# jhhung/kISS

Measured on AMD Instinct MI355X. Metric: bases/sec suffix_sort (chm13v2.0-size synthetic, k=256), higher is better.
Workload: dtype u8; 1 GPU; suffix_sort genome-like synthetic n=3117292070 k=256 (stand-in for chm13v2.0.fa, BASELINE.json configs[1]); PARALLEL_SORTING; text resident in HBM, SA left in HBM; n=3117292070, k=256, seed=2, parallelism=single GPU, lms=905939973, lms_rounds=9, tied_after_round0_item_rounds=184319413, big_segment_item_rounds=72866550, workspace_bytes=80357006484, induce_passes=47

## Files before the change

include/kiss_hip.h:

```cpp
#ifndef KISS_HIP_H
#define KISS_HIP_H

#include <stddef.h>
#include <stdint.h>

#ifdef __cplusplus
extern "C" {
#endif

#define KISS_HIP_VERSION 103

typedef enum kiss_hip_status {
    KISS_HIP_OK = 0,
    KISS_HIP_E_INVALID = -1,
    KISS_HIP_E_NO_DEVICE = -2,
    KISS_HIP_E_HIP = -3,
    KISS_HIP_E_NOMEM = -4,
    KISS_HIP_E_UNSUPPORTED = -5,
    KISS_HIP_E_INTERNAL = -6,
    KISS_HIP_E_IO = -7,
    KISS_HIP_E_DEEP = -8
} kiss_hip_status;

#define KISS_HIP_ALGO_PARALLEL_SORTING 0
// ... 75 lines not shown
int kiss_hip_release_cached_contexts(void);

int kiss_hip_ctx_suffix_sort_dna_u32(kiss_hip_ctx *ctx, const uint8_t *S, uint64_t n, uint32_t k, int algo,
                                     uint32_t *SA);

int kiss_hip_ctx_suffix_sort_dna_u32_dev(kiss_hip_ctx *ctx, const uint8_t *d_S, uint64_t n, uint32_t k, int algo,
                                         uint32_t *d_SA, void *stream);

typedef struct kiss_hip_multi kiss_hip_multi;
typedef struct kiss_hip_multi_stats {
    uint64_t n, m;
    uint32_t ndev;
    uint32_t refine_depth;
    uint64_t piece[8];
    float ms_total, ms_pack, ms_classify, ms_partition, ms_exchange, ms_sort, ms_gather, ms_induce;
} kiss_hip_multi_stats;
int kiss_hip_multi_create(kiss_hip_multi **out, const int *devices, int ndev, uint64_t max_n);
int kiss_hip_multi_destroy(kiss_hip_multi *mc);
int kiss_hip_multi_suffix_sort_dna_u32(kiss_hip_multi *mc, const uint8_t *S, uint64_t n, uint32_t k, int algo, uint32_t *SA);
int kiss_hip_multi_suffix_sort_dna_u32_dev(kiss_hip_multi *mc, const uint8_t *d_S, uint64_t n, uint32_t k, int algo,
                                           uint32_t *d_SA);
int kiss_hip_multi_get_stats(const kiss_hip_multi *mc, kiss_hip_multi_stats *out);
kiss_hip_ctx *kiss_hip_multi_ctx(kiss_hip_multi *mc, int rank);
int kiss_hip_suffix_sort_dna_u32_multi(const uint8_t *S, uint64_t n, uint32_t k, int algo, uint32_t *SA, const int *devices,
                                       int ndev);

typedef struct kiss_hip_verify_report {
    uint64_t n;
    uint32_t k;
    uint32_t exact;
    uint32_t ok;
    uint32_t sa0_ok;
    uint64_t out_of_range;
    uint64_t duplicates;
    uint64_t order_violations;
    uint64_t first_violation;
    uint64_t tied_pairs;
    uint64_t digest;
    float ms;
    uint32_t reserved_;
} kiss_hip_verify_report;
int kiss_hip_ctx_verify_sa_dev(kiss_hip_ctx *ctx, const uint8_t *d_S, uint64_t n, uint32_t k, const uint32_t *d_SA,
                               kiss_hip_verify_report *out, void *stream);
uint64_t kiss_hip_sa_digest_host(const uint32_t *SA, uint64_t count);
uint64_t kiss_hip_fnv1a64_host(const void *data, uint64_t bytes, uint64_t seed);

int kiss_hip_ctx_get_stage_outputs(kiss_hip_ctx *ctx, uint32_t *lms_ascending, uint32_t *lms_sorted,
                                   uint64_t *counts);

int kiss_hip_stage_classify(kiss_hip_ctx *ctx, const uint8_t *d_S, uint64_t n, uint32_t k, uint64_t lo, uint64_t hi,
                            uint64_t counts13[13], void *stream);
int kiss_hip_stage_local_lms(kiss_hip_ctx *ctx, uint64_t *d_keys_out ,
                             uint32_t *d_pos_out, uint64_t *m_local, uint64_t *m_far_local);
enum {
    KISS_HIP_VIEW_LOCAL_KEYS = 0,
    KISS_HIP_VIEW_LOCAL_POS = 1,
    KISS_HIP_VIEW_PART_KEYS = 2,
    KISS_HIP_VIEW_PART_POS = 3,
    KISS_HIP_VIEW_SORTED = 4,
    KISS_HIP_VIEW_SORTED_CTX = 5
};
int kiss_hip_stage_view(kiss_hip_ctx *ctx, int which, void **d_ptr, uint64_t *capacity);
int kiss_hip_stage_reserve(kiss_hip_ctx *ctx, uint64_t lms_capacity);
int kiss_hip_stage_key_hist(kiss_hip_ctx *ctx, const uint64_t *d_keys, uint64_t count, int bits, uint64_t *d_hist,
                            void *stream);
int kiss_hip_stage_partition(kiss_hip_ctx *ctx, const uint64_t *d_keys, const uint32_t *d_pos, uint64_t count, int bits,
                             const uint32_t *splitters, int groups, uint64_t *d_keys_out, uint32_t *d_pos_out,
                             void *stream);
int kiss_hip_stage_sort(kiss_hip_ctx *ctx, const uint64_t *d_keys, const uint32_t *d_pos, uint64_t count, uint64_t n,
                        uint32_t k, uint32_t *d_sorted_out, uint32_t *d_ctx_out, void *stream);
int kiss_hip_stage_induce(kiss_hip_ctx *ctx, uint64_t n, uint32_t k, const uint32_t *d_far_sorted,
                          const uint32_t *d_far_ctx, uint64_t m_far, const uint32_t *d_near_pos, uint64_t near_count,
                          const uint64_t counts12[12], uint32_t *d_SA, void *stream);
int kiss_hip_stage_induce_exact(kiss_hip_ctx *ctx, uint64_t n, uint32_t h0, const uint32_t *d_far_sorted,
                                const uint32_t *d_far_ctx, uint64_t m_far, const uint32_t *d_near_pos, uint64_t near_count,
                                const uint64_t counts12[12], uint32_t *d_SA, void *stream, int *exact_out);
int kiss_hip_stage_refine_exact(kiss_hip_ctx *ctx, uint64_t n, uint32_t h0, uint32_t *d_SA, void *stream);

int kiss_hip_debug_radix_sort(kiss_hip_ctx *ctx, uint64_t *keys, uint32_t *pos, uint64_t count, int key_lo_bit);
int kiss_hip_debug_radix_sort_seg(kiss_hip_ctx *ctx, uint64_t *keys, uint32_t *seg, uint32_t *pos, uint64_t count,
                                  int key_lo_bit, int seg_bits, unsigned flags);
int kiss_hip_debug_scan_u32(kiss_hip_ctx *ctx, uint32_t *data, uint64_t count);
int kiss_hip_debug_fail_alloc_over(kiss_hip_ctx *ctx, uint64_t bytes);
int kiss_hip_debug_splitters(const uint64_t *hist, uint64_t bins, int groups, uint32_t *splitters_out,
                             uint64_t *group_counts_out);

typedef struct kiss_hip_fmi_view {
    uint64_t n_sa;
    uint32_t cnt[4];
    uint32_t pri;
    uint32_t sa_intv;
    const uint8_t *bwt;
    const uint32_t *occ1;
    const uint8_t *occ2;
    const uint32_t *sa;
    const uint64_t *b;
    const uint32_t *b_occ;
} kiss_hip_fmi_view;

int kiss_hip_fmi_query_batch_dev(kiss_hip_ctx *ctx, const kiss_hip_fmi_view *fmi, const uint8_t *patterns, uint32_t L,
                                 uint64_t Q, uint32_t *beg, uint32_t *end, uint64_t *hit_count_total,
                                 uint64_t *checksum, uint32_t *offsets, uint64_t *offsets_index,
                                 uint64_t offsets_capacity, void *stream);

int kiss_hip_fmi_build_dev(kiss_hip_ctx *ctx, const uint8_t *d_S, uint64_t n, const uint32_t *d_SA, uint32_t sa_intv,
                           uint8_t *d_bwt, uint32_t *d_occ1, uint8_t *d_occ2, uint32_t *d_sa_sampled, uint64_t *d_b,
                           uint32_t *d_b_occ, uint32_t cnt_out[4], uint32_t *pri_out, void *stream);

typedef struct kiss_hip_fmi_sizes {
    uint64_t n_sa, bwt_bytes, occ1_entries, occ2_bytes, sa_entries, b_words, b_occ_entries;
} kiss_hip_fmi_sizes;
int kiss_hip_fmi_sizes_for(uint64_t n, kiss_hip_fmi_sizes *out);
int kiss_hip_fmi_build_host(const uint8_t *S, uint64_t n, const uint32_t *SA_or_null, uint8_t *bwt, uint32_t *occ1,
                            uint8_t *occ2, uint32_t *sa, uint64_t *b, uint32_t *b_occ, uint32_t cnt_out[4],
                            uint32_t *pri_out, int device);
int kiss_hip_fmi_query_batch_host(const kiss_hip_fmi_view *fmi, const uint8_t *patterns, uint32_t L, uint64_t Q,
                                  uint32_t *beg, uint32_t *end, uint64_t *hit_count_total, uint64_t *checksum,
                                  uint32_t *offsets, uint64_t *offsets_index, uint64_t offsets_capacity, int device);

#define KISS_HIP_FMI_MAX_SA_INTV 32u
#define KISS_HIP_FMI_MAX_LOOKUP_LEN 14u
typedef struct kiss_hip_fmi_view_ex {
    kiss_hip_fmi_view base;
    uint32_t lookup_len;
    const uint32_t *lookup;
} kiss_hip_fmi_view_ex;
typedef struct kiss_hip_fmi_sizes_ex {
    kiss_hip_fmi_sizes base;
    uint64_t lookup_entries;
} kiss_hip_fmi_sizes_ex;
int kiss_hip_fmi_sizes_ex_for(uint64_t n, uint32_t sa_intv, uint32_t lookup_len, kiss_hip_fmi_sizes_ex *out);
int kiss_hip_fmi_build_ex_dev(kiss_hip_ctx *ctx, const uint8_t *d_S, uint64_t n, const uint32_t *d_SA, uint32_t sa_intv,
                              uint32_t lookup_len, uint8_t *d_bwt, uint32_t *d_occ1, uint8_t *d_occ2, uint32_t *d_sa,
                              uint64_t *d_b, uint32_t *d_b_occ, uint32_t *d_lookup, uint32_t cnt_out[4], uint32_t *pri_out,
                              void *stream);
int kiss_hip_fmi_query_ex_dev(kiss_hip_ctx *ctx, const kiss_hip_fmi_view_ex *fmi, const uint8_t *patterns, uint32_t L,
                              uint64_t Q, uint32_t stop_cnt, uint32_t *beg, uint32_t *end, uint32_t *offs,
                              uint64_t *hit_count_total, uint64_t *checksum, uint32_t *offsets, uint64_t *offsets_index,
                              uint64_t offsets_capacity, void *stream);
int kiss_hip_fmi_build_ex_host(const uint8_t *S, uint64_t n, const uint32_t *SA_or_null, uint32_t sa_intv,
                               uint32_t lookup_len, uint8_t *bwt, uint32_t *occ1, uint8_t *occ2, uint32_t *sa, uint64_t *b,
                               uint32_t *b_occ, uint32_t *lookup, uint32_t cnt_out[4], uint32_t *pri_out, int device);
int kiss_hip_fmi_query_ex_host(const kiss_hip_fmi_view_ex *fmi, const uint8_t *patterns, uint32_t L, uint64_t Q,
                               uint32_t stop_cnt, uint32_t *beg, uint32_t *end, uint32_t *offs, uint64_t *hit_count_total,
                               uint64_t *checksum, uint32_t *offsets, uint64_t *offsets_index, uint64_t offsets_capacity,
                               int device);

#define KISS_HIP_FMI_MAX_MISMATCHES 3u
typedef struct kiss_hip_fmi_mm_report {
    uint64_t Q;
    uint32_t L, max_mismatches;
    uint64_t hits[4];
    uint64_t ranges;
    uint64_t lf_pairs;
    uint64_t walk_failures;
    uint64_t checksum;
    float ms_total, ms_search, ms_locate, ms_sort;
} kiss_hip_fmi_mm_report;
int kiss_hip_fmi_query_mm_dev(kiss_hip_ctx *ctx, const kiss_hip_fmi_view *fmi, const uint8_t *patterns, uint32_t L, uint64_t Q,
                              uint32_t max_mismatches, uint32_t *counts, uint32_t *positions, uint8_t *mismatches,
                              uint64_t *index, uint64_t capacity, kiss_hip_fmi_mm_report *report, void *stream);
int kiss_hip_fmi_query_mm_host(const kiss_hip_fmi_view *fmi, const uint8_t *patterns, uint32_t L, uint64_t Q,
                               uint32_t max_mismatches, uint32_t *counts, uint32_t *positions, uint8_t *mismatches,
                               uint64_t *index, uint64_t capacity, kiss_hip_fmi_mm_report *report, int device);

int kiss_hip_suffix_sort_u8(const uint8_t *S, uint64_t n, uint32_t *SA, int device);
// ... 207 lines not shown
```

kiss_amd/_lib.py:

```python
import ctypes
import os

_HERE = os.path.dirname(os.path.abspath(__file__))
LIB_PATH = os.path.join(_HERE, "libkiss_hip.so")
HOOKS_LIB_PATH = os.path.join(_HERE, "libkiss_hip_hooks.so")

KISS_HIP_OK = 0
KISS_HIP_E_INVALID, KISS_HIP_E_NO_DEVICE, KISS_HIP_E_HIP, KISS_HIP_E_NOMEM = -1, -2, -3, -4
KISS_HIP_E_UNSUPPORTED, KISS_HIP_E_INTERNAL, KISS_HIP_E_IO, KISS_HIP_E_DEEP = -5, -6, -7, -8
ALGO_PARALLEL_SORTING = 0
ALGO_PREFIX_DOUBLING = 1
MAX_N = 4294963200
VIEW_LOCAL_KEYS, VIEW_LOCAL_POS, VIEW_PART_KEYS, VIEW_PART_POS, VIEW_SORTED, VIEW_SORTED_CTX = range(6)

KERNEL_CLASSES = [
    "pack", "classify", "radix_hist", "radix_scatter", "scan", "keygather", "flag_compact",
    "place", "induce_count", "induce_scatter", "induce_small", "fm_query", "fm_build", "segrank",
    "group_heads", "isa",
]


class Report(ctypes.Structure):

    def as_dict(self):
# ... 265 lines not shown

class InsertReport(Report):
    _fields_ = [(k, ctypes.c_uint64) for k in ("P", "unmapped", "bad_input", "low_mapq", "discordant", "too_long", "samples", "used")] + [
        (k, ctypes.c_uint32) for k in ("flags", "q25", "q50", "q75", "mean", "sd", "ins_min", "ins_max", "ins_mean")] + [
        ("ms_total", ctypes.c_float), ("ms_hist", ctypes.c_float), ("ms_stats", ctypes.c_float),
    ]


class Fmi8View(ctypes.Structure):
    _fields_ = [
        ("n_sa", ctypes.c_uint64), ("pri", ctypes.c_uint32), ("sa_intv", ctypes.c_uint32), ("sigma", ctypes.c_uint32),
        ("reserved_", ctypes.c_uint32), ("C", ctypes.c_void_p), ("map", ctypes.c_void_p), ("bwt", ctypes.c_void_p),
        ("occ1", ctypes.c_void_p), ("occ2", ctypes.c_void_p), ("sa", ctypes.c_void_p), ("b", ctypes.c_void_p),
        ("b_occ", ctypes.c_void_p),
    ]


class Fmi8Sizes(Report):
    _fields_ = [(k, ctypes.c_uint64) for k in ("n_sa", "bwt_bytes", "occ1_entries", "occ2_entries", "sa_entries", "b_words",
                                               "b_occ_entries")]


class Fmi8Report(Report):
    _fields_ = [
        ("Q", ctypes.c_uint64), ("hits", ctypes.c_uint64), ("lf_pairs", ctypes.c_uint64), ("walk_failures", ctypes.c_uint64),
        ("checksum", ctypes.c_uint64), ("ms_total", ctypes.c_float), ("ms_search", ctypes.c_float),
        ("ms_locate", ctypes.c_float), ("ms_sort", ctypes.c_float),
    ]


class KissHipError(RuntimeError):
    def __init__(self, status, where, detail=""):
        self.status = status
        msg = "%s failed: %s (%d)" % (where, strerror(status), status)
        if detail:
            msg += " [" + detail + "]"
        super().__init__(msg)


_libs = {}


def load(hooks=None):
    if hooks is None:
        hooks = os.environ.get("KISS_AMD_LIB", "") == "hooks"
    hooks = bool(hooks)
    if hooks in _libs:
        return _libs[hooks]
    path = HOOKS_LIB_PATH if hooks else LIB_PATH
    if not hooks and os.environ.get("KISS_AMD_LIB_PATH"):
        path = os.environ["KISS_AMD_LIB_PATH"]
    if not os.path.exists(path):
        raise ImportError(
            "%s not built at %s -- run `python -c 'import __graft_entry__ as g; g.build()'` "
            "or `make -C kiss_amd/csrc`; there is no CPU fallback" % (os.path.basename(path), path))
    lib = ctypes.CDLL(path)
    if hasattr(lib, "kiss_hip_has_hooks"):
        lib.kiss_hip_has_hooks.restype = ctypes.c_int
        if bool(lib.kiss_hip_has_hooks()) != hooks and not os.environ.get("KISS_AMD_LIB_PATH"):
            raise ImportError("%s is not the %s build" % (path, "hooks" if hooks else "default"))
    elif hooks:
        raise ImportError("%s is not a hooks build" % path)
    vp, u8p = ctypes.c_void_p, ctypes.c_void_p
    lib.kiss_hip_version.restype = ctypes.c_int
    lib.kiss_hip_strerror.restype = ctypes.c_char_p
    lib.kiss_hip_strerror.argtypes = [ctypes.c_int]
    lib.kiss_hip_device_count.argtypes = [ctypes.POINTER(ctypes.c_int)]
    lib.kiss_hip_ctx_create.argtypes = [ctypes.POINTER(vp), ctypes.c_int, ctypes.c_uint64]
    lib.kiss_hip_ctx_create_sized.argtypes = [ctypes.POINTER(vp), ctypes.c_int, ctypes.c_uint64, ctypes.c_uint64]
    lib.kiss_hip_ctx_release_io_buffers.argtypes = [vp]
    ip = ctypes.POINTER(ctypes.c_int)
    lib.kiss_hip_multi_create.argtypes = [ctypes.POINTER(vp), ip, ctypes.c_int, ctypes.c_uint64]
    lib.kiss_hip_multi_destroy.argtypes = [vp]
    lib.kiss_hip_multi_suffix_sort_dna_u32.argtypes = [vp, vp, ctypes.c_uint64, ctypes.c_uint32, ctypes.c_int, vp]
    lib.kiss_hip_multi_suffix_sort_dna_u32_dev.argtypes = [vp, vp, ctypes.c_uint64, ctypes.c_uint32, ctypes.c_int, vp]
    lib.kiss_hip_multi_get_stats.argtypes = [vp, ctypes.POINTER(MultiStats)]
    lib.kiss_hip_multi_ctx.argtypes = [vp, ctypes.c_int]
    lib.kiss_hip_multi_ctx.restype = vp
    lib.kiss_hip_suffix_sort_dna_u32_multi.argtypes = [vp, ctypes.c_uint64, ctypes.c_uint32, ctypes.c_int, vp, ip, ctypes.c_int]
    lib.kiss_hip_stage_view.argtypes = [vp, ctypes.c_int, ctypes.POINTER(vp), ctypes.POINTER(ctypes.c_uint64)]
    lib.kiss_hip_stage_reserve.argtypes = [vp, ctypes.c_uint64]
    lib.kiss_hip_debug_fail_alloc_over.argtypes = [vp, ctypes.c_uint64]
    lib.kiss_hip_debug_fail_alloc_over.restype = ctypes.c_int
    lib.kiss_hip_debug_splitters.argtypes = [vp, ctypes.c_uint64, ctypes.c_int, vp, vp]
    lib.kiss_hip_debug_splitters.restype = ctypes.c_int
    lib.kiss_hip_ctx_destroy.argtypes = [vp]
    lib.kiss_hip_ctx_set_profiling.argtypes = [vp, ctypes.c_int]
    lib.kiss_hip_ctx_set_profiling_mask.argtypes = [vp, ctypes.c_uint64]
    lib.kiss_hip_last_hip_error.argtypes = [vp, ctypes.POINTER(ctypes.c_char_p)]
    lib.kiss_hip_get_stats.argtypes = [vp, ctypes.POINTER(Stats)]
    lib.kiss_hip_ctx_workspace_bytes.argtypes = [vp, ctypes.POINTER(ctypes.c_uint64)]
    lib.kiss_hip_suffix_sort_dna_u32.argtypes = [u8p, ctypes.c_uint64, ctypes.c_uint32, ctypes.c_int, vp, ctypes.c_int]
    lib.kiss_hip_ctx_suffix_sort_dna_u32.argtypes = [vp, u8p, ctypes.c_uint64, ctypes.c_uint32, ctypes.c_int, vp]
    lib.kiss_hip_ctx_suffix_sort_dna_u32_dev.argtypes = [vp, vp, ctypes.c_uint64, ctypes.c_uint32, ctypes.c_int, vp, vp]
    lib.kiss_hip_ctx_get_stage_outputs.argtypes = [vp, vp, vp, vp]
    lib.kiss_hip_ctx_verify_sa_dev.argtypes = [vp, vp, ctypes.c_uint64, ctypes.c_uint32, vp, ctypes.POINTER(VerifyReport), vp]
    lib.kiss_hip_ctx_verify_sa_dev.restype = ctypes.c_int
    lib.kiss_hip_sa_digest_host.argtypes = [vp, ctypes.c_uint64]
    lib.kiss_hip_sa_digest_host.restype = ctypes.c_uint64
    lib.kiss_hip_fnv1a64_host.argtypes = [vp, ctypes.c_uint64, ctypes.c_uint64]
    lib.kiss_hip_fnv1a64_host.restype = ctypes.c_uint64
    lib.kiss_hip_debug_radix_sort.argtypes = [vp, vp, vp, ctypes.c_uint64, ctypes.c_int]
    lib.kiss_hip_debug_radix_sort_seg.argtypes = [vp, vp, vp, vp, ctypes.c_uint64, ctypes.c_int, ctypes.c_int, ctypes.c_uint]
    lib.kiss_hip_debug_radix_sort_seg.restype = ctypes.c_int
    lib.kiss_hip_debug_scan_u32.argtypes = [vp, vp, ctypes.c_uint64]
    u64 = ctypes.c_uint64
    lib.kiss_hip_stage_classify.argtypes = [vp, vp, u64, ctypes.c_uint32, u64, u64, ctypes.POINTER(u64 * 13), vp]
    lib.kiss_hip_stage_local_lms.argtypes = [vp, vp, vp, ctypes.POINTER(u64), ctypes.POINTER(u64)]
    lib.kiss_hip_stage_key_hist.argtypes = [vp, vp, u64, ctypes.c_int, vp, vp]
    lib.kiss_hip_stage_partition.argtypes = [vp, vp, vp, u64, ctypes.c_int, vp, ctypes.c_int, vp, vp, vp]
    lib.kiss_hip_stage_sort.argtypes = [vp, vp, vp, u64, u64, ctypes.c_uint32, vp, vp, vp]
    lib.kiss_hip_stage_induce.argtypes = [vp, u64, ctypes.c_uint32, vp, vp, u64, vp, u64, ctypes.POINTER(u64 * 12), vp, vp]
    lib.kiss_hip_stage_induce_exact.argtypes = [vp, u64, ctypes.c_uint32, vp, vp, u64, vp, u64, ctypes.POINTER(u64 * 12), vp, vp,
                                                ctypes.POINTER(ctypes.c_int)]
    lib.kiss_hip_stage_refine_exact.argtypes = [vp, u64, ctypes.c_uint32, vp, vp]
    lib.kiss_hip_stage_refine_exact.restype = ctypes.c_int
    lib.kiss_hip_fmi_query_batch_dev.argtypes = [
        vp, ctypes.POINTER(FmiView), vp, ctypes.c_uint32, ctypes.c_uint64, vp, vp,
        ctypes.POINTER(ctypes.c_uint64), ctypes.POINTER(ctypes.c_uint64), vp, vp, ctypes.c_uint64, vp]
    lib.kiss_hip_fmi_build_dev.argtypes = [
        vp, vp, ctypes.c_uint64, vp, ctypes.c_uint32, vp, vp, vp, vp, vp, vp,
        ctypes.POINTER(ctypes.c_uint32 * 4), ctypes.POINTER(ctypes.c_uint32), vp]
    u32 = ctypes.c_uint32
    lib.kiss_hip_fmi_sizes_ex_for.argtypes = [u64, u32, u32, ctypes.POINTER(FmiSizesEx)]
    lib.kiss_hip_fmi_build_ex_dev.argtypes = [
        vp, vp, u64, vp, u32, u32, vp, vp, vp, vp, vp, vp, vp, ctypes.POINTER(u32 * 4), ctypes.POINTER(u32), vp]
    lib.kiss_hip_fmi_query_ex_dev.argtypes = [
        vp, ctypes.POINTER(FmiViewEx), vp, u32, u64, u32, vp, vp, vp, ctypes.POINTER(u64), ctypes.POINTER(u64), vp, vp,
        u64, vp]
    lib.kiss_hip_fmi_build_ex_host.argtypes = [vp, u64, vp, u32, u32] + [vp] * 9 + [ctypes.c_int]
    lib.kiss_hip_fmi_query_ex_host.argtypes = [ctypes.POINTER(FmiViewEx), vp, u32, u64, u32, vp, vp, vp,
                                               ctypes.POINTER(u64), ctypes.POINTER(u64), vp, vp, u64, ctypes.c_int]
    lib.kiss_hip_fmi_query_mm_dev.argtypes = [vp, ctypes.POINTER(FmiView), vp, u32, u64, u32, vp, vp, vp, vp, u64,
                                              ctypes.POINTER(FmiMmReport), vp]
    lib.kiss_hip_fmi_query_mm_host.argtypes = [ctypes.POINTER(FmiView), vp, u32, u64, u32, vp, vp, vp, vp, u64,
                                               ctypes.POINTER(FmiMmReport), ctypes.c_int]
    lib.kiss_hip_fmi_query_mm_dev.restype = lib.kiss_hip_fmi_query_mm_host.restype = ctypes.c_int
    lib.kiss_hip_fmi_seeds_dev.argtypes = [vp, ctypes.POINTER(FmiViewEx), vp, vp, u64, u32, u32, u32, ctypes.c_int, vp, vp, vp, u64,
                                           vp, vp, u64, ctypes.POINTER(FmiSeedReport), vp]
    lib.kiss_hip_fmi_seeds_host.argtypes = [ctypes.POINTER(FmiViewEx), vp, vp, u64, u32, u32, u32, ctypes.c_int, vp, vp, vp, u64,
                                            vp, vp, u64, ctypes.POINTER(FmiSeedReport), ctypes.c_int]
    lib.kiss_hip_fmi_seeds_dev.restype = lib.kiss_hip_fmi_seeds_host.restype = ctypes.c_int
    lib.kiss_hip_fmi_chain_dev.argtypes = [vp, vp, vp, u64, vp, vp, ctypes.POINTER(ChainParams), vp, vp, u64, vp, vp, u64,
                                           ctypes.POINTER(ChainReport), vp]
    lib.kiss_hip_fmi_chain_host.argtypes = [vp, vp, u64, vp, vp, ctypes.POINTER(ChainParams), vp, vp, u64, vp, vp, u64,
                                            ctypes.POINTER(ChainReport), ctypes.c_int]
    lib.kiss_hip_fmi_chain_dev.restype = lib.kiss_hip_fmi_chain_host.restype = ctypes.c_int
    lib.kiss_hip_fmi_align_dev.argtypes = [vp, vp, u64, vp, vp, u64, ctypes.c_int, vp, vp, ctypes.POINTER(AlignParams), vp, u64, vp,
                                           vp, u64, ctypes.POINTER(AlignReport), vp]
    lib.kiss_hip_fmi_align_host.argtypes = [vp, u64, vp, vp, u64, ctypes.c_int, vp, vp, ctypes.POINTER(AlignParams), vp, u64, vp, vp,
                                            u64, ctypes.POINTER(AlignReport), ctypes.c_int]
    lib.kiss_hip_fmi_align_dev.restype = lib.kiss_hip_fmi_align_host.restype = ctypes.c_int
    lib.kiss_hip_fmi_select_dev.argtypes = [vp, vp, vp, vp, u64, ctypes.c_int, vp, u64, ctypes.POINTER(SelectParams), vp, vp, u64,
                                            ctypes.POINTER(SelectReport), vp]
    lib.kiss_hip_fmi_select_host.argtypes = [vp, vp, vp, u64, ctypes.c_int, vp, u64, ctypes.POINTER(SelectParams), vp, vp, u64,
                                             ctypes.POINTER(SelectReport), ctypes.c_int]
    lib.kiss_hip_fmi_select_dev.restype = lib.kiss_hip_fmi_select_host.restype = ctypes.c_int
    lib.kiss_hip_fmi_pair_dev.argtypes = [vp, vp, vp, u64, vp, u64, ctypes.POINTER(PairParams), vp, ctypes.POINTER(PairReport), vp]
    lib.kiss_hip_fmi_pair_host.argtypes = [vp, vp, u64, vp, u64, ctypes.POINTER(PairParams), vp, ctypes.POINTER(PairReport),
                                           ctypes.c_int]
    lib.kiss_hip_fmi_pair_dev.restype = lib.kiss_hip_fmi_pair_host.restype = ctypes.c_int
    lib.kiss_hip_fmi_rescue_dev.argtypes = [vp, vp, vp, vp, u64, vp, u64, vp, u64, vp, u64, ctypes.POINTER(RescueParams), vp, vp, vp, u64,
                                            ctypes.POINTER(RescueReport), vp]
    lib.kiss_hip_fmi_rescue_host.argtypes = [vp, vp, vp, u64, vp, u64, vp, u64, vp, u64, ctypes.POINTER(RescueParams), vp, vp, vp, u64,
                                             ctypes.POINTER(RescueReport), ctypes.c_int]
    lib.kiss_hip_fmi_rescue_dev.restype = lib.kiss_hip_fmi_rescue_host.restype = ctypes.c_int
# ... 52 lines not shown
            getattr(lib, name).restype = ctypes.c_int
    lib.kiss_hip_fmi_insert_dev.argtypes = [vp, vp, vp, u64, vp, u64, ctypes.POINTER(InsertParams), vp, ctypes.POINTER(InsertReport), vp]
    lib.kiss_hip_fmi_insert_host.argtypes = [vp, vp, u64, vp, u64, ctypes.POINTER(InsertParams), vp, ctypes.POINTER(InsertReport),
                                             ctypes.c_int]
    for name in INSERT_EXPORTED_SYMBOLS:
        getattr(lib, name).restype = ctypes.c_int
    lib.kiss_hip_fmi8_sizes_for.argtypes = [u64, u32, u32, ctypes.POINTER(Fmi8Sizes)]
    lib.kiss_hip_fmi8_build_dev.argtypes = [vp, vp, u64, vp, u32, u32] + [vp] * 8 + [ctypes.POINTER(u32), ctypes.POINTER(u32), vp]
    lib.kiss_hip_fmi8_build_host.argtypes = [vp, u64, vp, u32, u32] + [vp] * 8 + [ctypes.POINTER(u32), ctypes.POINTER(u32),
                                                                                  ctypes.c_int]
    lib.kiss_hip_fmi8_query_dev.argtypes = [vp, ctypes.POINTER(Fmi8View), vp, vp, u64, vp, vp, ctypes.POINTER(u64),
                                            ctypes.POINTER(u64), vp, vp, u64, ctypes.POINTER(Fmi8Report), vp]
    lib.kiss_hip_fmi8_query_host.argtypes = [ctypes.POINTER(Fmi8View), vp, vp, u64, vp, vp, ctypes.POINTER(u64),
                                             ctypes.POINTER(u64), vp, vp, u64, ctypes.POINTER(Fmi8Report), ctypes.c_int]
    for name in ("kiss_hip_fmi8_sizes_for", "kiss_hip_fmi8_build_dev", "kiss_hip_fmi8_build_host", "kiss_hip_fmi8_query_dev",
                 "kiss_hip_fmi8_query_host"):
        getattr(lib, name).restype = ctypes.c_int
    lib.kiss_hip_file_size.argtypes = [ctypes.c_char_p, ctypes.POINTER(u64)]
    lib.kiss_hip_ctx_parse_text_dev.argtypes = [vp, vp, u64, vp, ctypes.POINTER(u64), vp]
    lib.kiss_hip_ctx_load_text_file.argtypes = [vp, ctypes.c_char_p, ctypes.POINTER(vp), ctypes.POINTER(u64)]
    lib.kiss_hip_copy_to_host.argtypes = [vp, vp, u64]
    lib.kiss_hip_suffix_sort_u8.argtypes = [vp, u64, vp, ctypes.c_int]
    lib.kiss_hip_suffix_sort_u8.restype = ctypes.c_int
    lib.kiss_hip_ctx_suffix_sort_u8_dev.argtypes = [vp, vp, u64, vp, vp]
    lib.kiss_hip_ctx_suffix_sort_u8_dev.restype = ctypes.c_int
    lib.kiss_hip_free_dev.argtypes = [vp]
    lib.kiss_hip_alloc_dev.argtypes = [ctypes.POINTER(vp), u64]
    lib.kiss_hip_alloc_dev.restype = ctypes.c_int
    for name in ("kiss_hip_ctx_lcp_dna_u32_dev", "kiss_hip_ctx_lcp_u8_dev"):
        getattr(lib, name).argtypes = [vp, vp, u64, vp, vp, ctypes.POINTER(LcpReport), vp]
        getattr(lib, name).restype = ctypes.c_int
    for name in ("kiss_hip_lcp_dna_u32", "kiss_hip_lcp_u8"):
        getattr(lib, name).argtypes = [vp, u64, vp, vp, vp, ctypes.c_int]
        getattr(lib, name).restype = ctypes.c_int
    for name in ("kiss_hip_file_size", "kiss_hip_ctx_parse_text_dev", "kiss_hip_ctx_load_text_file",
                 "kiss_hip_copy_to_host", "kiss_hip_free_dev"):
        getattr(lib, name).restype = ctypes.c_int
    for name in ("kiss_hip_device_count", "kiss_hip_ctx_create", "kiss_hip_ctx_destroy", "kiss_hip_ctx_set_profiling", "kiss_hip_ctx_set_profiling_mask",
                 "kiss_hip_last_hip_error", "kiss_hip_get_stats", "kiss_hip_ctx_workspace_bytes",
                 "kiss_hip_suffix_sort_dna_u32", "kiss_hip_ctx_suffix_sort_dna_u32",
                 "kiss_hip_ctx_suffix_sort_dna_u32_dev", "kiss_hip_ctx_get_stage_outputs",
                 "kiss_hip_fmi_query_batch_dev", "kiss_hip_fmi_build_dev", "kiss_hip_debug_radix_sort",
                 "kiss_hip_debug_scan_u32", "kiss_hip_stage_classify", "kiss_hip_stage_local_lms",
                 "kiss_hip_stage_key_hist", "kiss_hip_stage_partition", "kiss_hip_stage_sort", "kiss_hip_stage_induce",
                 "kiss_hip_ctx_create_sized", "kiss_hip_ctx_release_io_buffers", "kiss_hip_multi_create",
                 "kiss_hip_multi_destroy", "kiss_hip_multi_suffix_sort_dna_u32", "kiss_hip_multi_suffix_sort_dna_u32_dev",
                 "kiss_hip_multi_get_stats", "kiss_hip_suffix_sort_dna_u32_multi", "kiss_hip_stage_view",
                 "kiss_hip_stage_reserve", "kiss_hip_fmi_sizes_ex_for", "kiss_hip_fmi_build_ex_dev",
                 "kiss_hip_fmi_query_ex_dev", "kiss_hip_fmi_build_ex_host", "kiss_hip_fmi_query_ex_host"):
        getattr(lib, name).restype = ctypes.c_int
    _libs[hooks] = lib
    return lib


def strerror(status):
    return load().kiss_hip_strerror(int(status)).decode()


EXPORTED_SYMBOLS = [
    "kiss_hip_version", "kiss_hip_strerror", "kiss_hip_device_count", "kiss_hip_ctx_create", "kiss_hip_ctx_destroy",
    "kiss_hip_ctx_set_profiling", "kiss_hip_ctx_set_profiling_mask", "kiss_hip_last_hip_error", "kiss_hip_get_stats", "kiss_hip_ctx_workspace_bytes",
    "kiss_hip_suffix_sort_dna_u32", "kiss_hip_ctx_suffix_sort_dna_u32", "kiss_hip_ctx_suffix_sort_dna_u32_dev",
    "kiss_hip_ctx_get_stage_outputs", "kiss_hip_ctx_verify_sa_dev", "kiss_hip_sa_digest_host", "kiss_hip_fnv1a64_host",
    "kiss_hip_fmi_query_batch_dev", "kiss_hip_fmi_build_dev",
    "kiss_hip_debug_radix_sort", "kiss_hip_debug_radix_sort_seg", "kiss_hip_debug_scan_u32",
    "kiss_hip_stage_classify", "kiss_hip_stage_local_lms", "kiss_hip_stage_key_hist", "kiss_hip_stage_partition",
    "kiss_hip_stage_sort", "kiss_hip_stage_induce", "kiss_hip_stage_induce_exact", "kiss_hip_stage_refine_exact",
    "kiss_hip_fmi_sizes_for", "kiss_hip_fmi_build_host", "kiss_hip_fmi_query_batch_host",
    "kiss_hip_file_size", "kiss_hip_ctx_parse_text_dev", "kiss_hip_ctx_load_text_file", "kiss_hip_copy_to_host",
    "kiss_hip_free_dev", "kiss_hip_alloc_dev", "kiss_hip_suffix_sort_u8", "kiss_hip_ctx_suffix_sort_u8_dev",
    "kiss_hip_ctx_create_sized", "kiss_hip_ctx_release_io_buffers", "kiss_hip_stage_view", "kiss_hip_stage_reserve",
    "kiss_hip_multi_create", "kiss_hip_multi_destroy", "kiss_hip_multi_suffix_sort_dna_u32",
    "kiss_hip_multi_suffix_sort_dna_u32_dev", "kiss_hip_multi_get_stats", "kiss_hip_multi_ctx",
    "kiss_hip_suffix_sort_dna_u32_multi", "kiss_hip_debug_splitters", "kiss_hip_debug_fail_alloc_over",
    "kiss_hip_has_hooks", "kiss_hip_release_cached_contexts", "kiss_hip_get_stats_sized",
    "kiss_hip_fmi_sizes_ex_for", "kiss_hip_fmi_build_ex_dev", "kiss_hip_fmi_query_ex_dev", "kiss_hip_fmi_build_ex_host",
    "kiss_hip_fmi_query_ex_host", "kiss_hip_ctx_lcp_dna_u32_dev", "kiss_hip_ctx_lcp_u8_dev", "kiss_hip_lcp_dna_u32",
    "kiss_hip_lcp_u8", "kiss_hip_fmi_query_mm_dev", "kiss_hip_fmi_query_mm_host",
    "kiss_hip_fmi8_sizes_for", "kiss_hip_fmi8_build_dev", "kiss_hip_fmi8_build_host", "kiss_hip_fmi8_query_dev",
    "kiss_hip_fmi8_query_host", "kiss_hip_fmi_seeds_dev", "kiss_hip_fmi_seeds_host",
    "kiss_hip_fmi_chain_dev", "kiss_hip_fmi_chain_host", "kiss_hip_fmi_align_dev", "kiss_hip_fmi_align_host",
    "kiss_hip_fmi_select_dev", "kiss_hip_fmi_select_host", "kiss_hip_fmi_pair_dev", "kiss_hip_fmi_pair_host",
    "kiss_hip_fmi_rescue_dev", "kiss_hip_fmi_rescue_host", "kiss_hip_fmi_aln_merge_dev", "kiss_hip_fmi_aln_merge_host",
]

READS_EXPORTED_SYMBOLS = [
    "kiss_hip_reads_parse_dev", "kiss_hip_reads_parse_host", "kiss_hip_reads_interleave_dev", "kiss_hip_reads_interleave_host",
]
READS_PART_EXPORTED_SYMBOLS = ["kiss_hip_reads_parse_part_dev", "kiss_hip_reads_parse_part_host"]
MD_EXPORTED_SYMBOLS = ["kiss_hip_fmi_md_dev", "kiss_hip_fmi_md_host"]
PILEUP_EXPORTED_SYMBOLS = ["kiss_hip_fmi_pileup_dev", "kiss_hip_fmi_pileup_host"]
PILEUP_PLANES = 8
SAM_EXPORTED_SYMBOLS = ["kiss_hip_fmi_sam_dev", "kiss_hip_fmi_sam_host"]
BAM_EXPORTED_SYMBOLS = ["kiss_hip_fmi_bam_dev", "kiss_hip_fmi_bam_host", "kiss_hip_bgzf_dev", "kiss_hip_bgzf_host"]
BGZF_BLOCK_DEFAULT, BGZF_BLOCK_MAX, BGZF_OVERHEAD, BGZF_EOF_BYTES = 65280, 65505, 31, 28
DEFLATE_EXPORTED_SYMBOLS = ["kiss_hip_bgzf_deflate_dev", "kiss_hip_bgzf_deflate_host"]
BAM_SORT_EXPORTED_SYMBOLS = ["kiss_hip_bam_sort_dev", "kiss_hip_bam_sort_host"]
BAM_RECORD_MIN = 36
BAI_EXPORTED_SYMBOLS = ["kiss_hip_bai_dev", "kiss_hip_bai_host"]
BAI_PSEUDO_BIN, BAI_MAX_END = 37450, 1 << 29
INSERT_EXPORTED_SYMBOLS = ["kiss_hip_fmi_insert_dev", "kiss_hip_fmi_insert_host"]
INSERT_MAX = 65535
INSERT_OK = 1
READS_AUTO, READS_LINES, READS_FASTQ = 0, 1, 2
READS_NONE = 0xFFFFFFFFFFFFFFFF
```

kiss_amd/csrc/api.hip:

```cpp
#include "kiss_internal.hpp"
#include <cstdlib>
#include <chrono>
#include <mutex>
#include <cstring>
#include <new>

KTimer::KTimer(kiss_hip_ctx *c, int cls, uint64_t items) : ctx(c), idx(-1)
{
    if (!((ctx->profile_mask >> cls) & 1ull)) return;
    if (ctx->ev_used == ctx->ev_pool.size()) {
        kiss_hip_ctx::Ev e;
        if (hipEventCreate(&e.a) != hipSuccess || hipEventCreate(&e.b) != hipSuccess) return;
        e.cls = 0;
        ctx->ev_pool.push_back(e);
    }
    idx = (int)ctx->ev_used++;
    ctx->ev_pool[idx].cls = cls;
    ctx->stats.launches_kernel[cls]++;
    ctx->stats.items_kernel[cls] += items;
    (void)hipEventRecord(ctx->ev_pool[idx].a, ctx->stream);
}
KTimer::~KTimer()
{
    if (idx >= 0) (void)hipEventRecord(ctx->ev_pool[idx].b, ctx->stream);
}
void ktimer_collect(kiss_hip_ctx *ctx)
{
    for (size_t i = 0; i < ctx->ev_used; i++) {
        float ms = 0.f;
        if (hipEventElapsedTime(&ms, ctx->ev_pool[i].a, ctx->ev_pool[i].b) == hipSuccess)
            ctx->stats.ms_kernel[ctx->ev_pool[i].cls] += ms;
    }
    ctx->ev_used = 0;
}

static void kiss_opts_supported_from_env(KissOpts &o)
{
    o.debug = getenv("KISS_HIP_DEBUG") != nullptr;
    if (const char *e = getenv("KISS_HIP_XFER_THREADS")) o.xfer_threads = atoi(e);
    if (const char *e = getenv("KISS_HIP_PREFAULT_THREADS")) o.prefault_threads = atoi(e);
}
#ifdef KISS_HIP_HOOKS
static bool env_on(const char *name) { return getenv(name) != nullptr; }
static unsigned long long env_u64(const char *name, unsigned long long dflt)
{
    const char *e = getenv(name);
    return e ? strtoull(e, nullptr, 0) : dflt;
}
void kiss_opts_refresh(kiss_hip_ctx *ctx)
{
    KissOpts o;
    kiss_opts_supported_from_env(o);
    if (const char *e = getenv("KISS_HIP_SYNC_READBACK")) o.sync_readback = atoi(e) != 0;
    o.no_serialize = env_on("KISS_HIP_NO_SERIALIZE");
    o.no_lms_exact = env_on("KISS_HIP_NO_LMS_EXACT");
    o.heads_by_compare = env_on("KISS_HIP_LMS_HEADS_BY_COMPARE");
    o.no_early_out = env_on("KISS_HIP_NO_EARLY_OUT");
    o.no_pivot_rounds = env_on("KISS_HIP_NO_PIVOT_ROUNDS");
    o.pivot_from_round2 = env_on("KISS_HIP_PIVOT_FROM_ROUND2");
    o.pair_keys = env_on("KISS_HIP_PAIR_KEYS");
    o.no_fc0_onepass = env_on("KISS_HIP_NO_FC0_ONEPASS");
    o.no_pair_records = env_on("KISS_HIP_NO_PAIR_RECORDS");
    o.no_small_fused = env_on("KISS_HIP_NO_SMALL_FUSED");
    o.no_class_bytes = env_on("KISS_HIP_NO_CLASS_BYTES");
    o.no_pivot_ctx = env_on("KISS_HIP_NO_PIVOT_CTX");
    o.no_taint = env_on("KISS_HIP_NO_TAINT");
    o.isa_direct = env_on("KISS_HIP_ISA_DIRECT");
    o.no_onesweep = env_on("KISS_HIP_NO_ONESWEEP");
    o.rx_one_tile = env_on("KISS_HIP_RX_ONE_TILE");
    o.merge_lms = env_on("KISS_HIP_MERGE_LMS");
    o.no_small_alphabet = env_on("KISS_HIP_NO_SMALL_ALPHABET");
    o.induce_one_pass = env_on("KISS_HIP_INDUCE_ONE_PASS");
    o.verify = env_on("KISS_HIP_VERIFY");
    o.no_prefault = env_on("KISS_HIP_NO_PREFAULT");
    o.doubling_h0 = (uint32_t)env_u64("KISS_HIP_DOUBLING_H0", 0);
    o.tcap0 = env_u64("KISS_HIP_TCAP0", 0);
    o.pivot_slots = (int)env_u64("KISS_HIP_PIVOT_SLOTS", 3);
    o.small_seg = (uint32_t)env_u64("KISS_HIP_SMALL_SEG", 0);
    o.near_merge_min = (uint32_t)env_u64("KISS_HIP_NEAR_MERGE_MIN", 4096);
    o.induce_small_max = (uint32_t)env_u64("KISS_HIP_INDUCE_SMALL_MAX", 0);
    o.collapse_cap = (uint32_t)env_u64("KISS_HIP_COLLAPSE_CAP", 0);
    o.collapse_n = env_u64("KISS_HIP_COLLAPSE_N", 0);
    o.fm_heavy = (uint32_t)env_u64("KISS_HIP_FM_HEAVY", 0);
    o.fm_light = (uint32_t)env_u64("KISS_HIP_FM_LIGHT", 0);
    o.fm_mm_wave = env_on("KISS_HIP_FM_MM_WAVE");
    o.fm_mm_budget = env_u64("KISS_HIP_FM_MM_BUDGET", 0);
    o.fm8_group = env_on("KISS_HIP_FM8_GROUP");
    o.isa_direct_max = env_u64("KISS_HIP_ISA_DIRECT_MAX", 0);
    o.lx_sync_points = (unsigned)env_u64("KISS_HIP_LX_SYNC_POINTS", 0);
    o.tie_trace = (unsigned)env_u64("KISS_HIP_TIE_TRACE", 0);
    o.poison = (uint32_t)env_u64("KISS_HIP_POISON", 0);
    if (const char *e = getenv("KISS_HIP_DUMP_PIVOT")) snprintf(o.dump_pivot, sizeof o.dump_pivot, "%s", e);
    ctx->opts = o;
}
static std::mutex &kiss_launch_mutex()
{
    static std::mutex m;
    return m;
}
static bool kiss_lock_launches()
{
    static const bool on = getenv("KISS_HIP_LOCK_LAUNCHES") != nullptr;
    return on;
}
bool kiss_sync_launches()
{
    static const bool on = getenv("KISS_HIP_SYNC_LAUNCHES") != nullptr;
    return on;
}
KissLaunchGuard::KissLaunchGuard() : held(kiss_lock_launches())
{
    if (held) kiss_launch_mutex().lock();
}
KissLaunchGuard::~KissLaunchGuard()
{
    if (held) kiss_launch_mutex().unlock();
}
#endif

std::mutex &kiss_device_mutex(int device)
{
    static std::mutex m[64];
    return m[(unsigned)device & 63u];
}

__global__ void k_publish(const uint32_t *__restrict__ src, uint32_t nwords, uint32_t *host_dst, uint32_t seq)
{
    const uint32_t t = threadIdx.x;
    if (t < nwords) __hip_atomic_store(&host_dst[t], src[t], __ATOMIC_RELAXED, __HIP_MEMORY_SCOPE_SYSTEM);
    __threadfence_system();
    if (t == 0) __hip_atomic_store(&host_dst[16], seq, __ATOMIC_RELEASE, __HIP_MEMORY_SCOPE_SYSTEM);
}

int kiss_readback(kiss_hip_ctx *ctx, const void *d_src, uint32_t nwords)
{
    if (nwords > 16) return KINTERNAL();
    ctx->pub_mode = ctx->opts.sync_readback || !ctx->h_pub || !ctx->d_pub ? 0 : 1;
    if (ctx->pub_mode == 0) {
        KCHECK(hipMemcpyAsync(ctx->h_pinned, d_src, nwords * sizeof(uint32_t), hipMemcpyDeviceToHost, ctx->stream));
        KCHECK(hipStreamSynchronize(ctx->stream));
        return KISS_HIP_OK;
    }
    const uint32_t seq = ++ctx->pub_seq ? ctx->pub_seq : ++ctx->pub_seq;
    hipLaunchKernelGGL(k_publish, dim3(1), dim3(64), 0, ctx->stream, (const uint32_t *)d_src, nwords, ctx->d_pub, seq);
    KCHECK(hipGetLastError());
    volatile uint32_t *flag = ctx->h_pub + 16;
    const auto t0 = std::chrono::steady_clock::now();
    for (uint64_t spins = 0;; spins++) {
        if (__atomic_load_n(flag, __ATOMIC_ACQUIRE) == seq) break;
#if defined(__x86_64__) || defined(__i386__)
        __builtin_ia32_pause();
#endif
        if ((spins & 0xFFFF) == 0xFFFF) {
            const double s = std::chrono::duration<double>(std::chrono::steady_clock::now() - t0).count();
            if (s > 5.0) {
                KCHECK(hipStreamSynchronize(ctx->stream));
                if (__atomic_load_n(flag, __ATOMIC_ACQUIRE) != seq) return KINTERNAL();
                break;
            }
        }
    }
    for (uint32_t i = 0; i < nwords; i++) ctx->h_pinned[i] = ctx->h_pub[i];
    return KISS_HIP_OK;
}

bool kiss_host_is_pinned(const void *p);
void *kiss_prefault_start(kiss_hip_ctx *ctx, void *p, uint64_t bytes);
void kiss_prefault_join(void *handle);

void kiss_drain_deferred(kiss_hip_ctx *ctx)
{
    for (void *p : ctx->deferred_free) (void)hipFree(p);
    ctx->deferred_free.clear();
    ctx->deferred_bytes = 0;
}

namespace {

template <typename T>
int dmalloc(kiss_hip_ctx *ctx, T **p, uint64_t count)
{
    void *q = nullptr;
    uint64_t bytes = (count ? count : 1) * sizeof(T);
    hipError_t e = ctx->fail_alloc_over && bytes > ctx->fail_alloc_over ? hipErrorOutOfMemory : hipMalloc(&q, bytes);
#ifdef KISS_HIP_HOOKS
    if (e == hipSuccess && ctx->opts.poison) e = hipMemsetD32(q, (int)ctx->opts.poison, bytes / 4);
#endif
    if (e != hipSuccess) {
        (void)hipGetLastError();
        ctx->last_hip_error = (int)e;
        return KISS_HIP_E_NOMEM;
    }
    ctx->ws_bytes += bytes;
    *p = reinterpret_cast<T *>(q);
    return KISS_HIP_OK;
}

void release(kiss_hip_ctx *ctx, void *p, bool defer)
{
    if (defer) ctx->deferred_free.push_back(p);
    else (void)hipFree(p);
}

void free_tied(kiss_hip_ctx *ctx, bool defer = false)
{
    void **ptrs[] = {(void **)&ctx->segA, (void **)&ctx->segB, (void **)&ctx->slotA, (void **)&ctx->slotB,
                     (void **)&ctx->segstartA, (void **)&ctx->segstartB, (void **)&ctx->bkeyA, (void **)&ctx->bkeyB,
                     (void **)&ctx->bposA, (void **)&ctx->bposB, (void **)&ctx->bsegA, (void **)&ctx->bsegB,
                     (void **)&ctx->bslot, (void **)&ctx->flags};
    for (void **p : ptrs)
        if (*p) {
            release(ctx, *p, defer);
            *p = nullptr;
        }
    if (defer) ctx->deferred_bytes += ctx->tied_bytes;
    ctx->ws_bytes -= ctx->tied_bytes;
    ctx->tied_bytes = 0;
    ctx->t_cap = 0;
    ctx->flags_cap = 0;
}

void free_lms_side(kiss_hip_ctx *ctx, bool defer = false)
{
    free_tied(ctx, defer);
    void **ptrs[] = {(void **)&ctx->lms_pos, (void **)&ctx->keyA, (void **)&ctx->keyB, (void **)&ctx->posA,
                     (void **)&ctx->posB, (void **)&ctx->lms_sorted_far, (void **)&ctx->lms_ctx_far,
                     (void **)&ctx->lmsP, (void **)&ctx->lmsC, (void **)&ctx->tile_hist, (void **)&ctx->scan_tmp,
                     (void **)&ctx->rx_desc, (void **)&ctx->rx_ghist, (void **)&ctx->fc_desc};
    for (void **p : ptrs)
        if (*p) {
            release(ctx, *p, defer);
            *p = nullptr;
        }
    if (defer) ctx->deferred_bytes += ctx->lms_bytes;
    ctx->ws_bytes -= ctx->lms_bytes;
    ctx->lms_bytes = 0;
}

void free_all(kiss_hip_ctx *ctx)
{
    kiss_drain_deferred(ctx);
    free_lms_side(ctx);
    void *ptrs[] = {ctx->pk, ctx->tile_gp, ctx->tile_cnt, ctx->cl_part, ctx->d_counts, ctx->CTX, ctx->CLS, ctx->ind_counts, ctx->ind_desc,
                    ctx->d_small, ctx->near_idx, ctx->near_fin, ctx->near_pos, ctx->near_tmp, ctx->near_tmp2, ctx->pairs1, ctx->pairs2, ctx->rx_ctl, ctx->refine_heads, ctx->ga_codes};
    for (void *p : ptrs)
        if (p) (void)hipFree(p);
    for (void *p : ctx->fm_pool)
        if (p) (void)hipFree(p);
    for (hipEvent_t e : ctx->fm_ev)
        if (e) (void)hipEventDestroy(e);
#ifdef KISS_HIP_HOOKS
    if (ctx->tie_dbg) (void)hipFree(ctx->tie_dbg);
#endif
    if (ctx->io_S) (void)hipFree(ctx->io_S);
    if (ctx->io_SA) (void)hipFree(ctx->io_SA);
    kiss_xfer_free(ctx);
    if (ctx->h_pinned) (void)hipHostFree(ctx->h_pinned);
    if (ctx->h_pub) (void)hipHostFree(ctx->h_pub);
    for (auto &e : ctx->ev_pool) {
        (void)hipEventDestroy(e.a);
        (void)hipEventDestroy(e.b);
    }
    if (ctx->own_stream) (void)hipStreamDestroy(ctx->own_stream);
}

int sort_dev_unlocked(kiss_hip_ctx *ctx, const uint8_t *d_S, uint64_t n, uint32_t k, int algo, uint32_t *d_SA, void *stream);
int sort_dev(kiss_hip_ctx *ctx, const uint8_t *d_S, uint64_t n, uint32_t k, int algo, uint32_t *d_SA, void *stream)
{
    if (!ctx) return KISS_HIP_E_INVALID;
    kiss_opts_refresh(ctx);
#ifdef KISS_NO_DEVICE_LOCK
    return sort_dev_unlocked(ctx, d_S, n, k, algo, d_SA, stream);
#endif
    if (ctx->opts.no_serialize) return sort_dev_unlocked(ctx, d_S, n, k, algo, d_SA, stream);
    std::lock_guard<std::mutex> lock(kiss_device_mutex(ctx->device));
    return sort_dev_unlocked(ctx, d_S, n, k, algo, d_SA, stream);
}
int sort_dev_unlocked(kiss_hip_ctx *ctx, const uint8_t *d_S, uint64_t n, uint32_t k, int algo, uint32_t *d_SA, void *stream)
{
    if (!ctx || !d_SA || (n && !d_S)) return KISS_HIP_E_INVALID;
    if (n > KISS_HIP_MAX_N || n > ctx->max_n) return KISS_HIP_E_INVALID;
    if (algo != KISS_HIP_ALGO_PARALLEL_SORTING && algo != KISS_HIP_ALGO_PREFIX_DOUBLING) return KISS_HIP_E_INVALID;
    KCHECK(hipSetDevice(ctx->device));
    KissCallStream call_stream(ctx, stream);
    KTRY(kiss_workspace_ready(ctx));
    std::memset(&ctx->stats, 0, sizeof ctx->stats);
    ctx->stats.n = n;
    ctx->stats.k = k;
    ctx->n = n;
    ctx->m = ctx->m_far = 0;
    if (n == 0) {
        KTRY(kiss_zero_u32(ctx, d_SA, 1));
        KCHECK(hipStreamSynchronize(ctx->stream));
        return KISS_HIP_OK;
    }
    uint64_t depth;
    if ((uint64_t)k >= n) depth = 0;
    else depth = (uint64_t)KISS_STRIDE * ((uint64_t)k / KISS_STRIDE + 1);
    if (algo == KISS_HIP_ALGO_PREFIX_DOUBLING && depth != 0) {
        algo = KISS_HIP_ALGO_PARALLEL_SORTING;
    }
    ctx->stats.depth = (uint32_t)(depth > 0xFFFFFFFFull ? 0xFFFFFFFFull : depth);
    uint32_t h0 = 0;
    if (algo == KISS_HIP_ALGO_PREFIX_DOUBLING) {
        h0 = KISS_EXACT_H0;
        if (ctx->opts.doubling_h0 >= 32 && ctx->opts.doubling_h0 <= (1u << 20)) h0 = ctx->opts.doubling_h0;
        if (n < 4ull * h0 + 1024) h0 = 0;
        else {
            k = h0;
            depth = (uint64_t)KISS_STRIDE * ((uint64_t)k / KISS_STRIDE + 1);
        }
    }
    ctx->stats.refine_depth = h0;

    hipEvent_t ev[8];
    for (auto &e : ev) KCHECK(hipEventCreate(&e));
    const bool lms_exact = !ctx->opts.no_lms_exact;
    int rc = KISS_HIP_OK;
    for (int attempt = 0; attempt < 2; attempt++) {
        (void)hipEventRecord(ev[0], ctx->stream);
        if ((rc = kiss_pack_text(ctx, d_S, n))) break;
        (void)hipEventRecord(ev[1], ctx->stream);
        if ((rc = kiss_classify(ctx, n, depth, 0, n))) break;
        (void)hipEventRecord(ev[2], ctx->stream);
        ctx->hfar = nullptr;
        ctx->h_depth = h0;
// ... 262 lines not shown
    ctx->stats.ms_d2h = std::chrono::duration<float, std::milli>(t3 - t2).count();
    return KISS_HIP_OK;
}

int kiss_io_release(kiss_hip_ctx *ctx)
{
    if (ctx->io_S) (void)hipFree(ctx->io_S);
    if (ctx->io_SA) (void)hipFree(ctx->io_SA);
    ctx->io_S = nullptr;
    ctx->io_SA = nullptr;
    ctx->ws_bytes -= ctx->io_cap ? 5 * ctx->io_cap + 4 : 0;
    ctx->io_cap = 0;
    return KISS_HIP_OK;
}

extern "C" {

int kiss_hip_version(void) { return KISS_HIP_VERSION; }

const char *kiss_hip_strerror(int status)
{
    switch (status) {
    case KISS_HIP_OK: return "ok";
    case KISS_HIP_E_INVALID: return "invalid argument";
    case KISS_HIP_E_NO_DEVICE: return "no usable HIP device";
    case KISS_HIP_E_HIP: return "HIP runtime error";
    case KISS_HIP_E_NOMEM: return "out of memory";
    case KISS_HIP_E_UNSUPPORTED: return "request outside the implemented range";
    case KISS_HIP_E_INTERNAL: return "internal invariant violated";
    case KISS_HIP_E_IO: return "file could not be opened or read";
    case KISS_HIP_E_DEEP: return "ties deeper than the bounded-round exact path handles: sort with a bounded k, then stage_refine_exact";
    default: return "unknown status";
    }
}

int kiss_hip_device_count(int *count)
{
    if (!count) return KISS_HIP_E_INVALID;
    int c = 0;
    if (hipGetDeviceCount(&c) != hipSuccess) {
        *count = 0;
        return KISS_HIP_E_NO_DEVICE;
    }
    *count = c;
    return KISS_HIP_OK;
}

int kiss_hip_ctx_create(kiss_hip_ctx **out, int device, uint64_t max_n)
{
    return kiss_hip_ctx_create_sized(out, device, max_n, 0);
}

int kiss_hip_ctx_create_sized(kiss_hip_ctx **out, int device, uint64_t max_n, uint64_t lms_capacity)
{
    if (!out || max_n > KISS_HIP_MAX_N) return KISS_HIP_E_INVALID;
    *out = nullptr;
    int ndev = 0;
    if (hipGetDeviceCount(&ndev) != hipSuccess || ndev <= 0 || device < 0 || device >= ndev) return KISS_HIP_E_NO_DEVICE;
    kiss_hip_ctx *ctx = new (std::nothrow) kiss_hip_ctx();
    if (!ctx) return KISS_HIP_E_NOMEM;
    ctx->device = device;
    ctx->max_n = max_n;
    ctx->m_cap0 = lms_capacity ? lms_capacity + 4096 : 0;
    kiss_opts_supported_from_env(ctx->opts);
    kiss_opts_refresh(ctx);
    int rc = KISS_HIP_OK;
    do {
        if (hipSetDevice(device) != hipSuccess || hipStreamCreate(&ctx->own_stream) != hipSuccess) {
            rc = KISS_HIP_E_HIP;
            break;
        }
        ctx->stream = ctx->own_stream;
        const uint64_t words = max_n / 32 + 8;
        ctx->pk_words = words;
        ctx->n_tiles_cap = words / 256 + 2;
        ctx->ind_tiles_cap = 4 * ((max_n + 1) / 1024 + 2) + 2;
#define ALLOC(p, cnt) if ((rc = dmalloc(ctx, &ctx->p, (cnt)))) break
        ALLOC(pk, words);
        ALLOC(tile_gp, ctx->n_tiles_cap);
        ALLOC(tile_cnt, ctx->n_tiles_cap);
        ALLOC(cl_part, (ctx->n_tiles_cap < 8192 ? ctx->n_tiles_cap : 8192) * (uint64_t)(KISS_R0_PASSES * 256));
        ALLOC(d_counts, 16);
        ALLOC(ind_counts, ctx->ind_tiles_cap);
        ctx->ind_desc_stride = (max_n + 1) / 1024 + 2;
        ALLOC(ind_desc, 4 * ctx->ind_desc_stride);
        if (hipMemset(ctx->ind_desc, 0, 4 * ctx->ind_desc_stride * sizeof(uint64_t)) != hipSuccess) {
            rc = KISS_HIP_E_HIP;
            break;
        }
        ALLOC(rx_ctl, 4);
        if (hipMemset(ctx->rx_ctl, 0, 4 * sizeof(uint32_t)) != hipSuccess) {
            rc = KISS_HIP_E_HIP;
            break;
        }

        ALLOC(d_small, 64);
#undef ALLOC
        if ((rc = kiss_lms_reserve(ctx, default_m_cap(ctx)))) break;
        void *hp = nullptr;
        if (hipHostMalloc(&hp, 64 * sizeof(uint32_t), hipHostMallocDefault) != hipSuccess) {
            rc = KISS_HIP_E_NOMEM;
            break;
        }
        ctx->h_pinned = reinterpret_cast<uint32_t *>(hp);
        void *pub = nullptr, *dpub = nullptr;
        if (hipHostMalloc(&pub, 32 * sizeof(uint32_t), hipHostMallocCoherent | hipHostMallocMapped) == hipSuccess) {
            std::memset(pub, 0, 32 * sizeof(uint32_t));
            if (hipHostGetDevicePointer(&dpub, pub, 0) == hipSuccess) {
                ctx->h_pub = reinterpret_cast<uint32_t *>(pub);
                ctx->d_pub = reinterpret_cast<uint32_t *>(dpub);
            } else {
                (void)hipHostFree(pub);
            }
        }
        (void)hipGetLastError();
    } while (0);
    if (rc != KISS_HIP_OK) {
        free_all(ctx);
        delete ctx;
        return rc;
    }
    *out = ctx;
    return KISS_HIP_OK;
}

int kiss_hip_ctx_destroy(kiss_hip_ctx *ctx)
{
    if (!ctx) return KISS_HIP_E_INVALID;
    (void)hipSetDevice(ctx->device);
    free_all(ctx);
    delete ctx;
    return KISS_HIP_OK;
}

int kiss_hip_ctx_set_profiling(kiss_hip_ctx *ctx, int enabled)
{
    if (!ctx) return KISS_HIP_E_INVALID;
    ctx->profile_mask = enabled ? ~0ull : 0ull;
    return KISS_HIP_OK;
}

int kiss_hip_ctx_set_profiling_mask(kiss_hip_ctx *ctx, uint64_t class_mask)
{
    if (!ctx) return KISS_HIP_E_INVALID;
    ctx->profile_mask = class_mask;
    return KISS_HIP_OK;
}

int kiss_hip_last_hip_error(const kiss_hip_ctx *ctx, const char **msg)
{
    if (!ctx) return 0;
    if (msg) *msg = hipGetErrorString((hipError_t)ctx->last_hip_error);
    return ctx->last_hip_error;
}

int kiss_hip_get_stats(const kiss_hip_ctx *ctx, kiss_hip_stats *out)
{
    if (!ctx || !out) return KISS_HIP_E_INVALID;
    *out = ctx->stats;
    return KISS_HIP_OK;
}

int kiss_hip_get_stats_sized(const kiss_hip_ctx *ctx, void *out, uint64_t bytes)
{
    if (!ctx || !out) return KISS_HIP_E_INVALID;
    const uint64_t have = sizeof ctx->stats;
// ... 222 lines not shown
```

kiss_amd/csrc/induce.hip:

```cpp
#include "kiss_internal.hpp"
#include "induce_count.hpp"
#include <cstdio>
#include <cstdlib>

namespace {

constexpr int IN_THREADS = 256;
#ifndef KISS_IN_ITEMS
#define KISS_IN_ITEMS 8
#endif
constexpr int IN_ITEMS = KISS_IN_ITEMS;
constexpr int IN_WAVES = IN_THREADS / 64;
constexpr int IN_TILE = IN_THREADS * IN_ITEMS;
constexpr int SM_THREADS = 1024;
constexpr uint64_t SMALL_MAX = 8192;

__device__ __forceinline__ uint32_t child_ctx(uint32_t parent)
{
    return (KISS_CTX_WORD(parent) >> 2) | (parent & KISS_CTX_TAINT);
}

__device__ __forceinline__ uint32_t cls_byte(uint32_t c)
{
    return (c & 3u) | ((c & 0x7FFFFFFEu) == 0u ? 4u : 0u);
// ... 160 lines not shown
        const int nb = (int)mis - 4 * (int)lane;
        const uint32_t lowmask = nb >= 4 ? 0xFFFFFFFFu : (nb <= 0 ? 0u : ~(0xFFFFFFFFu << (8 * (nb & 3))));
        w[8] = (w[8] & lowmask) | (0x08080808u & ~lowmask);
    }
    KissClsAcc acc = {{0u, 0u, 0u, 0u}};
    uint32_t any = 0;
#pragma unroll
    for (int i = 0; i < 8; i++) {
        kiss_cls_acc_add(acc, w[i]);
        any |= w[i];
    }
    if (mis != 0u) {
        kiss_cls_acc_add(acc, w[8]);
        any |= w[8];
    }
    uint32_t cnt8 = kiss_cls_acc_sum(acc);
    if (__ballot((any & 0x04040404u) != 0u) != 0ull) {
        uint64_t pend = 0;
#pragma unroll
        for (int i = 0; i < 9; i++) {
            const uint32_t p = (w[i] >> 2) & ~(w[i] >> 3) & 0x01010101u;
            pend |= (uint64_t)(((p * 0x00204081u) >> 21) & 0xFu) << (4 * i);
        }
        cnt8 = refresh_pending<4>(pk, srcP, srcC, srcK, pend, first + 16 * (int64_t)lane, 1024, first + 2048 + 4 * (int64_t)lane,
                                  cnt8, false);
    }
    put_counts(counts, tiles, tile, kiss_cls_emit(cnt8, emitmask));
}

__device__ __forceinline__ void count_word_tile(const uint64_t *__restrict__ pk, const uint32_t *srcP, uint32_t *srcC, int64_t beg,
                                                int dir, uint32_t emitmask, uint32_t *__restrict__ counts, uint64_t tiles,
                                                uint64_t tile, int64_t shift)
{
    struct __attribute__((packed, aligned(4))) U4 {
        uint32_t v[4];
    };
    constexpr int STEPS = IN_TILE / 256;
    static_assert(STEPS * 4 == 32, "one bit per item of a lane in the low half of refresh_pending's mask");
    static_assert(IN_TILE / 64 <= 255, "8-bit counters per lane");
    const uint64_t i0 = tile * IN_TILE + 4 * lane_id();
    const int64_t p0 = (dir > 0 ? beg + (int64_t)i0 : beg - (int64_t)(i0 + 3)) - shift;
    const int64_t pstep = dir > 0 ? 256 : -256;
    U4 t[STEPS];
#pragma unroll
    for (int q = 0; q < STEPS; q++) t[q] = *reinterpret_cast<const U4 *>(srcC + (p0 + q * pstep));
    uint32_t cnt8 = 0, least = 0xFFFFFFFFu;
#pragma unroll
    for (int q = 0; q < STEPS; q++) {
#pragma unroll
        for (int e = 0; e < 4; e++) {
            cnt8 += 1u << ((t[q].v[e] << 3) & 31u);
            least = min(least, t[q].v[e] & 0x7FFFFFFEu);
        }
    }
    if (__ballot(least == 0u) != 0ull) {
        uint32_t pend = 0;
#pragma unroll
        for (int q = 0; q < STEPS; q++)
#pragma unroll
            for (int e = 0; e < 4; e++) pend |= ((t[q].v[e] & 0x7FFFFFFEu) == 0u ? 1u : 0u) << (4 * q + e);
        cnt8 = refresh_pending<2>(pk, srcP, srcC, nullptr, (uint64_t)pend, p0, pstep, 0, cnt8, true);
    }
    put_counts(counts, tiles, tile, kiss_cls_emit(cnt8, emitmask));
}

template <bool REMAP>
__device__ __forceinline__ void count_partial_tile(const uint64_t *__restrict__ pk, const uint32_t *srcP, uint32_t *srcC, int64_t beg,
                                                   uint64_t N, int dir, uint32_t emitmask, uint32_t *__restrict__ counts,
                                                   uint64_t tiles, uint64_t tile, const LmsRemap &rm, uint8_t *srcK)
{
    const uint64_t t0 = tile * IN_TILE;
    uint32_t cnt8 = 0;
    for (uint64_t i = t0 + lane_id(); i < N && i < t0 + IN_TILE; i += 64) {
        const uint32_t cls = item_class_only<REMAP>(pk, srcP, srcC, beg + (int64_t)dir * (int64_t)i, emitmask, rm, REMAP ? nullptr : srcK);
        cnt8 += (cls < 4u ? 1u : 0u) << ((cls & 3u) << 3);
    }
    put_counts(counts, tiles, tile, cnt8);
}

template <bool REMAP>
__global__ __launch_bounds__(IN_THREADS) void k_induce_count(const uint64_t *__restrict__ pk, const uint32_t *srcP,
                                                            uint32_t *srcC, int64_t beg, uint64_t N, int dir,
                                                            uint32_t emitmask, uint32_t *__restrict__ counts,
                                                            uint64_t tiles, LmsRemap rm, uint8_t *srcK)
{
    if (blockIdx.x == 0 && threadIdx.x == 4) counts[4 * tiles] = 0;
    const uint32_t wave = (uint32_t)__builtin_amdgcn_readfirstlane((int)(threadIdx.x >> 6));
    const uint64_t tile = (uint64_t)blockIdx.x * IN_WAVES + wave;
    if (tile >= tiles) return;
    const uint64_t t0 = tile * IN_TILE;
    int64_t shift = 0;
    bool block = t0 + IN_TILE <= N;
    if (REMAP && block) {
        const uint32_t b0 = remap_below_wave(rm, (uint64_t)beg + t0);
        block = b0 == remap_below_wave(rm, (uint64_t)beg + t0 + IN_TILE);
        shift = (int64_t)b0;
    }
    if (!block) count_partial_tile<REMAP>(pk, srcP, srcC, beg, N, dir, emitmask, counts, tiles, tile, rm, srcK);
    else if (!REMAP && srcK != nullptr) count_byte_tile(pk, srcP, srcC, srcK, beg, dir, emitmask, counts, tiles, tile);
    else count_word_tile(pk, srcP, srcC, beg, dir, emitmask, counts, tiles, tile, shift);
}

struct DstPos {
    int64_t p[4];
};

template <bool REMAP, int DIR>
__global__ __launch_bounds__(IN_THREADS) void k_induce_scatter(const uint64_t *__restrict__ pk, const uint32_t *srcP,
                                                              uint32_t *srcC, int64_t beg, uint64_t N,
                                                              uint32_t emitmask, const uint32_t *__restrict__ ex,
                                                              uint64_t tiles, DstPos dst, uint32_t *SA, uint32_t *CTX,
                                                              uint32_t *__restrict__ totals, LmsRemap rm,
                                                              uint8_t *CLS,
                                                              uint8_t *srcK)
{
    static_assert(IN_ITEMS == 8 && IN_WAVES == 4, "8-bit counters per thread, 4-bit ranks of a thread's items in one word");
    static_assert(!REMAP || DIR > 0, "the LMS list is read left to right only");
    __shared__ uint32_t wtot[IN_WAVES][2];
    __shared__ __attribute__((aligned(16))) uint32_t stP[IN_TILE];
    __shared__ __attribute__((aligned(16))) uint32_t stC[IN_TILE];
    if (blockIdx.x == 0 && threadIdx.x < 4) totals[threadIdx.x] = ex[(uint64_t)(threadIdx.x + 1) * tiles] - ex[(uint64_t)threadIdx.x * tiles];
    const int wave = threadIdx.x >> 6;
    struct __attribute__((packed, aligned(4))) U4 {
        uint32_t v[4];
    };
    const uint64_t i0 = (uint64_t)blockIdx.x * IN_TILE + (uint64_t)threadIdx.x * IN_ITEMS;
    uint32_t vv[IN_ITEMS], cc[IN_ITEMS];
    uint32_t okm = 0;
    uint32_t loc = 0;
    uint32_t cnt8 = 0;
    auto take = [&](int e, uint32_t pc, uint32_t ok) {
        const uint32_t sh = pc << 3;
        loc |= ((cnt8 >> sh) & 15u) << (4 * e);
        cnt8 += ok << sh;
        okm |= ok << e;
    };
    int64_t shift = 0;
    bool block = i0 + IN_ITEMS <= N;
    if (REMAP) {
        const uint64_t tj = (uint64_t)beg + (uint64_t)blockIdx.x * IN_TILE;
        const uint32_t t0 = remap_below_wave(rm, tj), t1 = remap_below_wave(rm, tj + IN_TILE);
        if (t0 == t1) shift = (int64_t)t0;
        else if (block) {
            const uint32_t b0 = remap_below(rm, (uint64_t)beg + i0);
            block = b0 == remap_below(rm, (uint64_t)beg + i0 + IN_ITEMS);
            shift = (int64_t)b0;
        }
    }
    if (block) {
        const int64_t p0 = (DIR > 0 ? beg + (int64_t)i0 : beg - (int64_t)(i0 + IN_ITEMS - 1)) - shift;
        uint32_t bp[IN_ITEMS], bc[IN_ITEMS];
#pragma unroll
        for (int q = 0; q < IN_ITEMS / 4; q++) {
            const U4 tp = *reinterpret_cast<const U4 *>(srcP + p0 + 4 * q);
            const U4 tcw = *reinterpret_cast<const U4 *>(srcC + p0 + 4 * q);
#pragma unroll
            for (int e = 0; e < 4; e++) {
                bp[4 * q + e] = tp.v[e];
                bc[4 * q + e] = tcw.v[e];
            }
        }
        uint32_t least = 0xFFFFFFFFu;
#pragma unroll
        for (int e = 0; e < IN_ITEMS; e++) least = min(least, bc[e] & 0x7FFFFFFEu);
        static_assert(KISS_EMPTY_CTX == 1u && KISS_CTX_TAINT == 0x80000000u, "no bases <=> all bits but 0 and 31 clear");
        constexpr int last = IN_ITEMS - 1;
        if (__ballot(least == 0u) == 0ull) {
#pragma unroll
            for (int e = 0; e < IN_ITEMS; e++) {
                const int a = DIR > 0 ? e : last - e;
                const uint32_t pc = bc[a] & 3u;
                take(e, pc, (emitmask >> pc) & 1u);
// ... 320 lines not shown
}

template <bool REMAP>
__global__ __launch_bounds__(SM_THREADS) void k_induce_small(const uint64_t *__restrict__ pk, const uint32_t *srcP0,
                                                            uint32_t *srcC0, int64_t beg0, uint64_t N0, int dir,
                                                            uint32_t emitmask, int selfclass, DstPos dst, uint32_t *SA,
                                                            uint32_t *CTX, uint32_t *out, LmsRemap rm, uint8_t *CLS)
{
    __shared__ int64_t heads[4];
    __shared__ uint32_t wtot[SM_THREADS / 64][4];
    __shared__ uint32_t chunk_tot[4];
    __shared__ uint32_t round_self;
    if (threadIdx.x < 4) heads[threadIdx.x] = dst.p[threadIdx.x];
    if (threadIdx.x == 0) round_self = 0;
    __syncthreads();

    const uint32_t *srcP = srcP0;
    uint32_t *srcC = srcC0;
    int64_t beg = beg0;
    uint64_t N = N0;
    uint32_t rounds = 0;
    const int wave = threadIdx.x >> 6;

    while (N > 0) {
        rounds++;
        const int64_t self_head_at_start = selfclass >= 0 ? heads[selfclass] : 0;
        __syncthreads();
        for (uint64_t cb = 0; cb < N; cb += SM_THREADS) {
            uint64_t i = cb + threadIdx.x;
            uint32_t cls = 4u, v = 0, cw = 0;
            if (i < N) cls = item_class<REMAP>(pk, srcP, srcC, beg + (int64_t)dir * (int64_t)i, emitmask, &v, &cw, rm);
            uint32_t myrank = 0;
            uint32_t tot[4];
#pragma unroll
            for (int c = 0; c < 4; c++) {
                uint64_t mk = __ballot(cls == (uint32_t)c);
                if (cls == (uint32_t)c) myrank = (uint32_t)__popcll(mk & lanemask_lt());
                tot[c] = (uint32_t)__popcll(mk);
            }
            if (lane_id() == 0) {
#pragma unroll
                for (int c = 0; c < 4; c++) wtot[wave][c] = tot[c];
            }
            __syncthreads();
            if (cls < 4u) {
                uint32_t o = myrank;
                for (int w = 0; w < wave; w++) o += wtot[w][cls];
                int64_t d = heads[cls] + (int64_t)dir * (int64_t)o;
                SA[d] = v - 1u;
                CTX[d] = child_ctx(cw);
                if (CLS) CLS[d] = (uint8_t)cls_byte(child_ctx(cw));
            }
            if (threadIdx.x < 4) {
                uint32_t t = 0;
                for (int w = 0; w < SM_THREADS / 64; w++) t += wtot[w][threadIdx.x];
                chunk_tot[threadIdx.x] = t;
            }
            __syncthreads();
            if (threadIdx.x < 4) heads[threadIdx.x] += (int64_t)dir * (int64_t)chunk_tot[threadIdx.x];
            if (threadIdx.x == 0 && selfclass >= 0) round_self += chunk_tot[selfclass];
            __syncthreads();
        }
        if (selfclass < 0) break;
        uint64_t nextN = round_self;
        __syncthreads();
        if (threadIdx.x == 0) round_self = 0;
        srcP = SA;
        srcC = CTX;
        beg = self_head_at_start;
        N = nextN;
        __syncthreads();
    }
    if (threadIdx.x < 4) out[threadIdx.x] = (uint32_t)((heads[threadIdx.x] - dst.p[threadIdx.x]) * (int64_t)dir);
    if (threadIdx.x == 0) out[4] = rounds;
}

struct Sweep {
    kiss_hip_ctx *ctx;
    uint32_t *SA;
    int dir;
    int64_t pos[4];
};

int run_pass(Sweep &sw, const uint32_t *srcP, uint32_t *srcC, int64_t beg, uint64_t N, uint32_t emitmask,
             int selfclass, uint64_t tot[4], bool *chain_done, const LmsRemap *remap = nullptr)
{
    kiss_hip_ctx *ctx = sw.ctx;
    const LmsRemap rm = remap ? *remap : LmsRemap{nullptr, nullptr, 0u};
    if (remap && (sw.dir < 0 || selfclass >= 0)) return KINTERNAL();
    for (int c = 0; c < 4; c++) tot[c] = 0;
    *chain_done = false;
    if (N == 0 || emitmask == 0) {
        *chain_done = true;
        return KISS_HIP_OK;
    }
    DstPos dp;
    for (int c = 0; c < 4; c++) dp.p[c] = sw.pos[c];
    ctx->stats.induce_passes++;
    uint8_t *const srcK = (srcC == ctx->CTX && ctx->CLS && !ctx->opts.no_class_bytes && !ctx->opts.induce_one_pass) ? ctx->CLS : nullptr;
    const uint64_t small_max = ctx->opts.induce_small_max >= 64 && ctx->opts.induce_small_max <= (1u << 20) ? ctx->opts.induce_small_max
                                                                                                           : (uint64_t)SMALL_MAX;
    if (N <= small_max) {
        {
            KTimer t(ctx, KISS_HIP_K_INDUCE_SMALL, N);
            if (remap)
                hipLaunchKernelGGL(k_induce_small<true>, dim3(1), dim3(SM_THREADS), 0, ctx->stream, ctx->pk, srcP, srcC, beg, N,
                                   sw.dir, emitmask, selfclass, dp, sw.SA, ctx->CTX, ctx->d_small, rm, ctx->CLS);
            else
                hipLaunchKernelGGL(k_induce_small<false>, dim3(1), dim3(SM_THREADS), 0, ctx->stream, ctx->pk, srcP, srcC, beg, N,
                                   sw.dir, emitmask, selfclass, dp, sw.SA, ctx->CTX, ctx->d_small, rm, ctx->CLS);
            KCHECK(hipGetLastError());
        }
        KTRY(kiss_readback(ctx, ctx->d_small, 5));
        for (int c = 0; c < 4; c++) tot[c] = ctx->h_pinned[c];
        *chain_done = true;
    } else {
        const uint64_t tiles = div_up(N, IN_TILE);
        if (4 * tiles + 1 > ctx->ind_tiles_cap) return KINTERNAL();
#ifdef KISS_HIP_HOOKS
        if (ctx->opts.induce_one_pass && ctx->ind_desc && tiles <= ctx->ind_desc_stride && tiles < (1ull << 31)) {
            KTimer t(ctx, KISS_HIP_K_INDUCE_SCATTER, N);
            ctx->ind_epoch++;
            if (remap)
                hipLaunchKernelGGL(k_induce_onepass<true>, dim3((unsigned)tiles), dim3(IN_THREADS), 0, ctx->stream, ctx->pk, srcP,
                                   srcC, beg, N, sw.dir, emitmask, tiles, dp, sw.SA, ctx->CTX, ctx->d_small, rm, ctx->ind_desc,
                                   ctx->ind_desc_stride, ctx->rx_ctl, ctx->ind_ticket_base, ctx->ind_epoch);
            else
                hipLaunchKernelGGL(k_induce_onepass<false>, dim3((unsigned)tiles), dim3(IN_THREADS), 0, ctx->stream, ctx->pk, srcP,
                                   srcC, beg, N, sw.dir, emitmask, tiles, dp, sw.SA, ctx->CTX, ctx->d_small, rm, ctx->ind_desc,
                                   ctx->ind_desc_stride, ctx->rx_ctl, ctx->ind_ticket_base, ctx->ind_epoch);
            KCHECK(hipGetLastError());
            ctx->ind_ticket_base += (uint32_t)tiles;
        } else
#endif
        {
        {
            KTimer t(ctx, KISS_HIP_K_INDUCE_COUNT, N);
            if (remap)
                hipLaunchKernelGGL(k_induce_count<true>, dim3((unsigned)div_up(tiles, IN_WAVES)), dim3(IN_THREADS), 0, ctx->stream,
                                   ctx->pk, srcP, srcC, beg, N, sw.dir, emitmask, ctx->ind_counts, tiles, rm, srcK);
            else
                hipLaunchKernelGGL(k_induce_count<false>, dim3((unsigned)div_up(tiles, IN_WAVES)), dim3(IN_THREADS), 0, ctx->stream,
                                   ctx->pk, srcP, srcC, beg, N, sw.dir, emitmask, ctx->ind_counts, tiles, rm, srcK);
            KCHECK(hipGetLastError());
        }
        KTRY(kiss_scan_u32(ctx, ctx->ind_counts, ctx->ind_counts, 4 * tiles + 1));
        {
            KTimer t(ctx, KISS_HIP_K_INDUCE_SCATTER, N);
            if (remap)
                hipLaunchKernelGGL((k_induce_scatter<true, 1>), dim3((unsigned)tiles), dim3(IN_THREADS), 0, ctx->stream, ctx->pk, srcP,
                                   srcC, beg, N, emitmask, ctx->ind_counts, tiles, dp, sw.SA, ctx->CTX, ctx->d_small, rm, ctx->CLS, srcK);
            else if (sw.dir > 0)
                hipLaunchKernelGGL((k_induce_scatter<false, 1>), dim3((unsigned)tiles), dim3(IN_THREADS), 0, ctx->stream, ctx->pk, srcP,
                                   srcC, beg, N, emitmask, ctx->ind_counts, tiles, dp, sw.SA, ctx->CTX, ctx->d_small, rm, ctx->CLS, srcK);
            else
                hipLaunchKernelGGL((k_induce_scatter<false, -1>), dim3((unsigned)tiles), dim3(IN_THREADS), 0, ctx->stream, ctx->pk, srcP,
                                   srcC, beg, N, emitmask, ctx->ind_counts, tiles, dp, sw.SA, ctx->CTX, ctx->d_small, rm, ctx->CLS, srcK);
            KCHECK(hipGetLastError());
        }
        }
        KTRY(kiss_readback(ctx, ctx->d_small, 4));
        for (int c = 0; c < 4; c++) tot[c] = ctx->h_pinned[c];
    }
    if (ctx->opts.debug)
        fprintf(stderr, "[kiss_hip] pass dir=%d beg=%lld N=%llu mask=%x self=%d -> %llu,%llu,%llu,%llu\n", sw.dir, (long long)beg,
                (unsigned long long)N, emitmask, selfclass, (unsigned long long)tot[0], (unsigned long long)tot[1],
                (unsigned long long)tot[2], (unsigned long long)tot[3]);
    for (int c = 0; c < 4; c++) sw.pos[c] += (int64_t)sw.dir * (int64_t)tot[c];
    return KISS_HIP_OK;
}

constexpr uint64_t COLLAPSE_N = 1ull << 18;
constexpr uint32_t COLLAPSE_RCAP = 65535;
constexpr uint32_t COLLAPSE_RCAP_WIDE = (1u << 22) - 1;
constexpr int CH_THREADS = 256;

constexpr uint32_t RUN_SERIAL = 1024;

__device__ __forceinline__ uint32_t run_before(const uint64_t *__restrict__ pk, uint64_t v, uint32_t c, uint32_t cap,
                                               bool valid)
{
    const uint64_t pat = (uint64_t)c * 0x5555555555555555ull;
    const uint32_t scap = cap < RUN_SERIAL ? cap : RUN_SERIAL;
    uint32_t r = 0;
    uint64_t p = valid ? v : 0;
    bool going = false;
    while (p > 0) {
        const uint64_t q = p - 1;
        const uint32_t in = (uint32_t)(q & 31u) + 1u;
        const uint64_t y = (pk[q >> 5] ^ pat) >> (62u - 2u * (uint32_t)(q & 31u));
        uint32_t mt = y ? (uint32_t)(__ffsll((unsigned long long)y) - 1) >> 1 : 32u;
        if (mt > in) mt = in;
        r += mt;
        p -= mt;
        if (mt < in) break;
        if (r >= scap) {
            going = r < cap && p > 0;
            break;
        }
    }
    uint64_t todo = __ballot(going);
    while (todo) {
        const int leader = __ffsll((unsigned long long)todo) - 1;
        todo &= todo - 1;
        uint64_t lp = __shfl(p, leader, 64);
        uint32_t lr = __shfl(r, leader, 64);
        const uint32_t lcap = __shfl(cap, leader, 64);
        while (true) {
            const int64_t w = (int64_t)(lp >> 5) - 1 - (int64_t)lane_id();
            const uint64_t y = w >= 0 ? (pk[w] ^ pat) : 1ull;
            const uint64_t stop = __ballot(y != 0);
            if (!stop) {
                lr += 2048u;
                lp -= 2048u;
                if (lr >= lcap) break;
                continue;
            }
            const int f = __ffsll((unsigned long long)stop) - 1;
            const uint64_t yf = __shfl(y, f, 64);
            const bool outside = ((int64_t)(lp >> 5) - 1 - f) < 0;
            lr += 32u * (uint32_t)f + (outside ? 0u : ((uint32_t)(__ffsll((unsigned long long)yf) - 1) >> 1));
            break;
        }
        if ((int)lane_id() == leader) r = lr;
    }
    return r > cap ? cap : r;
}

__global__ __launch_bounds__(CH_THREADS) void k_chain_runs(const uint64_t *__restrict__ pk, const uint32_t *srcP,
                                                          const uint32_t *srcC, int64_t beg, uint64_t N, int dir, uint32_t c,
                                                          uint32_t cap,
                                                          int rshift, uint32_t termmask, uint32_t *__restrict__ run,
                                                          uint64_t *__restrict__ tkey, uint32_t *__restrict__ tpos,
                                                          uint32_t *__restrict__ counters)
{
    uint64_t i = (uint64_t)blockIdx.x * CH_THREADS + threadIdx.x;
    uint32_t cls = 4u;
    bool capped = false;
    const uint64_t v = i < N ? srcP[beg + (int64_t)dir * (int64_t)i] : 0;
    const uint32_t r = run_before(pk, v, c, cap, i < N);
// ... 156 lines not shown
                td.p[x] = sw.pos[x];
                td.off[x] = o;
                o += cnt[x];
            }
            td.off[4] = o;
            KTimer t(ctx, KISS_HIP_K_INDUCE_SMALL, T);
            hipLaunchKernelGGL(k_chain_term_write, dim3((unsigned)div_up(T, CH_THREADS)), dim3(CH_THREADS), 0,
                               ctx->stream, ctx->pk, tb.key[res], tb.pos[res], T, td, sw.dir, sw.SA, ctx->CTX, ctx->CLS);
            KCHECK(hipGetLastError());
        }
        for (int x = 0; x < 4; x++) sw.pos[x] += (int64_t)sw.dir * (int64_t)cnt[x];
        sw.pos[c] += (int64_t)sw.dir * (int64_t)E;
        beg = dst + (int64_t)sw.dir * (int64_t)(E - ncap);
        N = ncap;
        wide = cap >= COLLAPSE_RCAP;
    }
    return KISS_HIP_OK;
}

__global__ void k_checksum(const uint64_t *__restrict__ pk, uint64_t words, unsigned long long *out)
{
    uint64_t i = (uint64_t)blockIdx.x * blockDim.x + threadIdx.x;
    unsigned long long v = 0;
    for (; i < words; i += (uint64_t)gridDim.x * blockDim.x) v += pk[i] * (2 * i + 1);
    for (int d = 32; d >= 1; d >>= 1) v += __shfl_xor(v, d, 64);
    if (lane_id() == 0) atomicAdd(out, v);
}
int checksum_pk(kiss_hip_ctx *ctx, const char *what)
{
    unsigned long long *d = (unsigned long long *)(ctx->d_small + 60);
    KTRY(kiss_zero_u32(ctx, d, 2));
    hipLaunchKernelGGL(k_checksum, dim3(256), dim3(256), 0, ctx->stream, ctx->pk, ctx->n / 32 + 2, d);
    unsigned long long h = 0;
    KCHECK(hipMemcpyAsync(&h, d, 8, hipMemcpyDeviceToHost, ctx->stream));
    KCHECK(hipStreamSynchronize(ctx->stream));
    fprintf(stderr, "[kiss_hip] pk checksum %016llx at %s\n", h, what);
    return KISS_HIP_OK;
}

__global__ void k_verify_part(const uint64_t *__restrict__ pk, const uint32_t *SA, const uint32_t *CTX, int64_t lo,
                              int64_t hi, uint32_t c, uint64_t n, uint32_t *bad)
{
    int64_t i = lo + (int64_t)blockIdx.x * blockDim.x + threadIdx.x;
    if (i >= hi) return;
    uint32_t v = SA[i], cw = KISS_CTX_WORD(CTX[i]);
    bool ok = v < n && kiss_base(pk, v) == c;
    if (ok && cw != KISS_EMPTY_CTX) {
        uint32_t full = kiss_load_ctx(pk, v);
        int mb = 31 - __clz(cw);
        uint32_t mask = (1u << mb) - 1u;
        ok = (mb % 2 == 0) && mb <= 30 && ((full & mask) == (cw & mask)) && (31 - __clz(full)) >= mb;
    }
    if (!ok) {
        uint32_t k = atomicAdd(&bad[0], 1u);
        if (k < 6) {
            bad[1 + 3 * k] = (uint32_t)i;
            bad[2 + 3 * k] = v;
            bad[3 + 3 * k] = cw;
        }
    }
}

int verify_part(kiss_hip_ctx *ctx, const uint32_t *SA, int64_t lo, int64_t hi, uint32_t c, uint64_t n, const char *what)
{
    if (hi <= lo) return KISS_HIP_OK;
    uint32_t *bad = ctx->d_small + 40;
    KTRY(kiss_zero_u32(ctx, bad, 20));
    hipLaunchKernelGGL(k_verify_part, dim3((unsigned)div_up((uint64_t)(hi - lo), 256)), dim3(256), 0, ctx->stream, ctx->pk,
                       SA, ctx->CTX, lo, hi, c, n, bad);
    uint32_t h[20];
    KCHECK(hipMemcpyAsync(h, bad, sizeof h, hipMemcpyDeviceToHost, ctx->stream));
    KCHECK(hipStreamSynchronize(ctx->stream));
    fprintf(stderr, "[kiss_hip] verify %s c=%u [%lld,%lld): bad %u", what, c, (long long)lo, (long long)hi, h[0]);
    for (uint32_t k = 0; k < h[0] && k < 6; k++) fprintf(stderr, " (idx %u v %u ctx %08x)", h[1 + 3 * k], h[2 + 3 * k], h[3 + 3 * k]);
    fprintf(stderr, "\n");
    return KISS_HIP_OK;
}

}

int kiss_induce(kiss_hip_ctx *ctx, uint64_t n, uint32_t *d_SA)
{
    ctx->stats.induce_passes = 0;
    KTRY(kiss_need_ctx_words(ctx));
    ctx->ctx_words_valid = false;
    uint64_t cnt[4], cntS[4], cntL[4], cntLMS[4], start[5], lms_start[5];
    start[0] = 1;
    lms_start[0] = 0;
    for (int c = 0; c < 4; c++) {
        cnt[c] = ctx->counts[c];
        cntS[c] = ctx->counts[4 + c];
        cntLMS[c] = ctx->counts[8 + c];
        cntL[c] = cnt[c] - cntS[c];
        start[c + 1] = start[c] + cnt[c];
        lms_start[c + 1] = lms_start[c] + cntLMS[c];
    }
    if (start[4] != n + 1) return KINTERNAL();

    uint32_t *seed = ctx->d_small + 32;
    ctx->h_pinned[32] = (uint32_t)n;
    ctx->h_pinned[33] = KISS_EMPTY_CTX;
    KCHECK(hipMemcpyAsync(seed, ctx->h_pinned + 32, 2 * sizeof(uint32_t), hipMemcpyHostToDevice, ctx->stream));
    KCHECK(hipMemcpyAsync(d_SA, ctx->h_pinned + 32, sizeof(uint32_t), hipMemcpyHostToDevice, ctx->stream));
    KCHECK(hipStreamSynchronize(ctx->stream));

    uint64_t tot[4];
    bool done;
    if (ctx->opts.verify) KTRY(checksum_pk(ctx, "induce start"));
    const uint64_t collapse_n = ctx->opts.collapse_n >= 1024 && ctx->opts.collapse_n <= (1ull << 26) ? ctx->opts.collapse_n : (uint64_t)COLLAPSE_N;
    uint64_t collapse_max = collapse_n < ctx->m_cap ? collapse_n : ctx->m_cap;
    if (collapse_max > ctx->t_cap) collapse_max = ctx->t_cap;

    const LmsRemap lms_rm{ctx->rm_fin, ctx->rm_pos, ctx->rm_E};
    Sweep L{ctx, d_SA, +1, {(int64_t)start[0], (int64_t)start[1], (int64_t)start[2], (int64_t)start[3]}};
    KTRY(run_pass(L, seed, seed + 1, 0, 1, 0xFu, -1, tot, &done));
    for (int c = 0; c < 4; c++) {
        int64_t a = (int64_t)start[c];
        const uint32_t mask_ge = (0xFu << c) & 0xFu;
        while (L.pos[c] > a) {
            uint64_t N = (uint64_t)(L.pos[c] - a);
            if (N <= collapse_max) {
                KTRY(run_collapse(L, (uint32_t)c, a, N, mask_ge));
                a = L.pos[c];
                break;
            }
            KTRY(run_pass(L, d_SA, ctx->CTX, a, N, mask_ge, c, tot, &done));
            a = done ? L.pos[c] : a + (int64_t)N;
        }
        if ((uint64_t)L.pos[c] != start[c] + cntL[c]) return KINTERNAL();
        KTRY(kiss_early_out(ctx, d_SA, c == 0 ? 0 : start[c], start[c] + cntL[c]));
        if (cntLMS[c]) {
            const uint32_t mask_gt = (0xFu << (c + 1)) & 0xFu;
            if (ctx->lms_merged) KTRY(run_pass(L, ctx->lmsP, ctx->lmsC, (int64_t)lms_start[c], cntLMS[c], mask_gt, -1, tot, &done));
            else KTRY(run_pass(L, ctx->lms_sorted_far, ctx->lms_ctx_far, (int64_t)lms_start[c], cntLMS[c], mask_gt, -1, tot, &done, &lms_rm));
        }
    }

    if (ctx->opts.verify) KTRY(checksum_pk(ctx, "L sweep end"));
    if (ctx->opts.verify)
        for (int c = 0; c < 4; c++) KTRY(verify_part(ctx, d_SA, (int64_t)start[c], (int64_t)(start[c] + cntL[c]), (uint32_t)c, n, "L-part"));
    Sweep S{ctx, d_SA, -1, {(int64_t)start[1] - 1, (int64_t)start[2] - 1, (int64_t)start[3] - 1, (int64_t)start[4] - 1}};
    for (int c = 3; c >= 0; c--) {
        int64_t hi = (int64_t)start[c + 1];
        const uint32_t mask_le = (1u << (c + 1)) - 1u;
        while (S.pos[c] + 1 < hi) {
            uint64_t N = (uint64_t)(hi - (S.pos[c] + 1));
            if (N <= collapse_max) {
                KTRY(run_collapse(S, (uint32_t)c, hi - 1, N, mask_le));
                hi = S.pos[c] + 1;
                break;
            }
            KTRY(run_pass(S, d_SA, ctx->CTX, hi - 1, N, mask_le, c, tot, &done));
            hi = done ? S.pos[c] + 1 : hi - (int64_t)N;
        }
        if ((uint64_t)(S.pos[c] + 1) != start[c] + cntL[c]) {
            fprintf(stderr, "[kiss_hip] S sweep bucket %d: tail %lld, expected %llu\n", c, (long long)(S.pos[c] + 1),
                    (unsigned long long)(start[c] + cntL[c]));
            return KINTERNAL();
        }
        KTRY(kiss_early_out(ctx, d_SA, start[c] + cntL[c], start[c + 1]));
        if (cntL[c] && c > 0) {
            const uint32_t mask_lt = (1u << c) - 1u;
            KTRY(run_pass(S, d_SA, ctx->CTX, (int64_t)(start[c] + cntL[c]) - 1, cntL[c], mask_lt, -1, tot, &done));
        }
    }
    ctx->ctx_words_valid = true;
    return KISS_HIP_OK;
}
```

kiss_amd/csrc/kiss_internal.hpp:

```cpp
#pragma once
#include <hip/hip_runtime.h>
#include <stdint.h>
#include <stddef.h>
#include <mutex>
#include <vector>
#include "../../include/kiss_hip.h"

struct KissOpts {
    bool debug = false;
    int xfer_threads = 0;
    int prefault_threads = 0;
    bool sync_readback = false;
    bool no_lms_exact = false;
    bool heads_by_compare = false;
    bool no_early_out = false;
    bool no_pivot_rounds = false;
    bool pivot_from_round2 = false;
    bool pair_keys = false;
    bool no_fc0_onepass = false;
    bool no_pair_records = false;
    bool no_small_fused = false;
    bool no_class_bytes = false;
    bool no_pivot_ctx = false;
    bool no_taint = false;
    bool isa_direct = false;
    bool no_onesweep = false;
    bool rx_one_tile = false;
    bool merge_lms = false;
    bool no_small_alphabet = false;
    bool induce_one_pass = false;
    bool verify = false;
    bool no_prefault = false;
    bool no_serialize = false;
    bool lock_launches = false;
    bool sync_launches = false;
    uint32_t doubling_h0 = 0;
    uint64_t tcap0 = 0;
    int pivot_slots = 3;
    uint32_t small_seg = 0;
    uint32_t near_merge_min = 4096;
    uint32_t induce_small_max = 0;
    uint32_t collapse_cap = 0;
    uint64_t collapse_n = 0;
    uint32_t fm_heavy = 0, fm_light = 0;
    bool fm_mm_wave = false;
    bool fm8_group = false;
    uint64_t fm_mm_budget = 0;
    uint64_t isa_direct_max = 0;
    unsigned lx_sync_points = 0;
    unsigned tie_trace = 0;
    uint32_t poison = 0;
    char dump_pivot[256] = {0};
};
struct kiss_hip_ctx;
#ifdef KISS_HIP_HOOKS
void kiss_opts_refresh(kiss_hip_ctx *ctx);
struct KissLaunchGuard {
    bool held;
    KissLaunchGuard();
    ~KissLaunchGuard();
};
bool kiss_sync_launches();
#define KISS_ARG4_(a, b, c, d, ...) d
#ifdef hipLaunchKernelGGL
#undef hipLaunchKernelGGL
#define hipLaunchKernelGGL(kernelName, ...)                                                                            \
    do {                                                                                                               \
        KissLaunchGuard kiss_launch_guard_;                                                                            \
        hipLaunchKernelGGLInternal((kernelName), __VA_ARGS__);                                                         \
        if (kiss_sync_launches()) (void)hipStreamSynchronize(KISS_ARG4_(__VA_ARGS__, 0, 0, 0, 0));                     \
    } while (0)
#endif
#else
static inline void kiss_opts_refresh(kiss_hip_ctx *) {}
#endif

#define KISS_EMPTY_CTX 1u
#define KISS_CTX_BASES 15u
#define KISS_CTX_TAINT 0x80000000u
#define KISS_CTX_WORD(c) ((c) & 0x7FFFFFFFu)
#define KISS_STRIDE 125u

#define KCHECK(call)                                   \
    do {                                               \
        hipError_t e__ = (call);                       \
        if (e__ != hipSuccess) {                       \
            ctx->last_hip_error = (int)e__;            \
            return (e__ == hipErrorOutOfMemory) ? KISS_HIP_E_NOMEM : KISS_HIP_E_HIP; \
        }                                              \
    } while (0)
#define KTRY(expr)                 \
    do {                           \
        int s__ = (expr);          \
        if (s__ != KISS_HIP_OK) return s__; \
    } while (0)

#include <cstdio>
#define KINTERNAL() (fprintf(stderr, "[kiss_hip] internal check failed at %s:%d\n", __FILE__, __LINE__), KISS_HIP_E_INTERNAL)

enum FmSlot {
    FM_SLOT_HEAVY,
    FM_SLOT_CAP,
    FM_SLOT_CAP_INDEX,
    FM_SLOT_GOT,
    FM_SLOT_GOT_INDEX,
    FM_SLOT_TOTALS,
    FM_SLOT_FRONTIER0,
    FM_SLOT_FRONTIER1,
    FM_SLOT_OFFSETS,
    FM_SLOT_FCAP,
    FM_SLOT_FCAP_INDEX,
    FM_SLOT_BLOCKS,
    FM_SLOT_MEDIUM,
    FM_SLOT_MM_CTL,
    FM_SLOT_MM_LEAVES,
    FM_SLOT_MM_QTOT,
    FM_SLOT_MM_LEAF_SIZE,
    FM_SLOT_MM_LEAF_INDEX,
    FM_SLOT_MM_HEAVY,
    FM_SLOT_MM_HFLAG,
    FM_SLOT_FM8_CTL,
    FM_SLOT_FM8_COUNTS,
    FM_SLOT_SEED_CTL,
    FM_SLOT_SEED_MS,
    FM_SLOT_SEED_RANGES,
    FM_SLOT_SEED_FLAGS,
    FM_SLOT_SEED_SCANNED,
    FM_SLOT_SEED_POS_SIZE,
    FM_SLOT_CHAIN_CTL,
    FM_SLOT_CHAIN_SLAB,
    FM_SLOT_CHAIN_VSTART,
    FM_SLOT_ALIGN_CTL,
    FM_SLOT_ALIGN_SLAB,
    FM_SLOT_ALIGN_TRACE,
    FM_SLOT_SELECT_CTL,
    FM_SLOT_SELECT_SLAB,
// ... 5 lines not shown
    FM_SLOT_READS_LINES,
    FM_SLOT_READS_INDEX,
    FM_SLOT_MD_CTL,
    FM_SLOT_MD_SLAB,
    FM_SLOT_INSERT_CTL,
    FM_SLOT_INSERT_HIST,
    FM_SLOT_SAM_CTL,
    FM_SLOT_SAM_READS,
    FM_SLOT_SAM_LINES,
    FM_SLOT_PILEUP_CTL,
    FM_SLOT_DEFLATE_TOKENS,
    FM_SLOT_DEFLATE_STAGE,
    FM_SLOT_DEFLATE_SIZES,
    FM_SLOT_BAM_SORT_CTL,
    FM_SLOT_BAM_SORT_INDEX,
    FM_SLOT_BAI_CTL,
    FM_SLOT_BAI_REC,
    FM_SLOT_BAI_REF,
    FM_SLOT_BAI_WIN,
    FM_SLOT_BAI_ITEMS,
    FM_SLOT_COUNT
};

struct kiss_hip_ctx {
    int device = 0;
    int last_hip_error = 0;
    KissOpts opts;
#ifdef KISS_HIP_HOOKS
    uint32_t *tie_dbg = nullptr;
    bool tie_dbg_on = false;
    uint32_t tie_dbg_E = 0, tie_dbg_k = 0;
#endif
    hipStream_t own_stream = nullptr;
    hipStream_t stream = nullptr;
    uint64_t max_n = 0;
    uint64_t m_cap = 0;
    uint64_t fail_alloc_over = 0;
    uint64_t m_cap0 = 0;
    uint64_t t_cap = 0;
    uint64_t flags_cap = 0;
    uint64_t tied_bytes = 0;
    uint64_t ws_bytes = 0;
    uint64_t lms_bytes = 0;
    std::vector<void *> deferred_free;
    uint64_t deferred_bytes = 0;

    uint64_t *pk = nullptr;
    uint64_t pk_words = 0;
    uint32_t *tile_gp = nullptr;
    uint32_t *tile_cnt = nullptr;
    uint8_t *CLS = nullptr;
    uint32_t *cl_part = nullptr;
    uint64_t n_tiles_cap = 0;
    uint32_t *d_counts = nullptr;
    uint32_t *lms_pos = nullptr;
    bool lms_pos_complete = false;
    uint64_t *keyA = nullptr, *keyB = nullptr;
    uint32_t *posA = nullptr, *posB = nullptr;
    uint32_t *segA = nullptr, *segB = nullptr;
    uint32_t *slotA = nullptr, *slotB = nullptr;
    uint32_t *segstartA = nullptr, *segstartB = nullptr;
    uint64_t *bkeyA = nullptr, *bkeyB = nullptr;
    uint32_t *bposA = nullptr, *bposB = nullptr, *bsegA = nullptr, *bsegB = nullptr, *bslot = nullptr;
    uint64_t *flags = nullptr;
    uint32_t *lms_sorted_far = nullptr;
    uint32_t *lms_ctx_far = nullptr;
    uint32_t *lmsP = nullptr;
    uint32_t *lmsC = nullptr;
    uint32_t *tile_hist = nullptr;
    uint64_t tile_hist_cap = 0;
    uint64_t *rx_desc = nullptr;
    uint32_t *rx_ghist = nullptr, *rx_ctl = nullptr;
    uint64_t rx_ghist_count = 0;
    uint64_t rx_tiles_cap = 0, rx_epoch = 0;
    uint64_t *fc_desc = nullptr;
    uint64_t fc_desc_cap = 0;
    uint32_t rx_ticket_base = 0;
    uint64_t *scan_tmp = nullptr;
    uint64_t scan_tmp_cap = 0;
    uint32_t *CTX = nullptr;
    bool ctx_words_valid = false;
    uint32_t *ind_counts = nullptr;
    uint64_t ind_tiles_cap = 0;
    uint64_t *ind_desc = nullptr;
    uint64_t ind_desc_stride = 0, ind_epoch = 0;
    uint32_t ind_ticket_base = 0;
    uint32_t *d_small = nullptr;
    uint32_t *h_pinned = nullptr;
    uint32_t *h_pub = nullptr;
    uint32_t *d_pub = nullptr;
    uint32_t pub_seq = 0;
    int pub_mode = -1;
    uint64_t *pairs1 = nullptr, *pairs2 = nullptr;
    uint64_t pairs_cap = 0;
    void *fm_pool[FM_SLOT_COUNT] = {};
    uint64_t fm_pool_cap[FM_SLOT_COUNT] = {};
    int cu_count = 0;
    hipEvent_t fm_ev[6] = {};
    uint32_t *near_idx = nullptr, *near_fin = nullptr, *near_pos = nullptr, *near_tmp = nullptr, *near_tmp2 = nullptr;
    uint64_t near_cap = 0;
    uint8_t *ga_codes = nullptr;
    uint64_t ga_codes_cap = 0;
    uint8_t *refine_heads = nullptr;
    uint8_t *hfar = nullptr, *hmerged = nullptr;
    uint32_t h_depth = 0;
    bool lms_merged = false;
    int near_form = 0;
    const uint32_t *near_sorted = nullptr;
    const uint32_t *rm_fin = nullptr, *rm_pos = nullptr;
    uint32_t rm_E = 0;

    uint8_t *io_S = nullptr;
    uint32_t *io_SA = nullptr;
    uint64_t io_cap = 0;
    uint32_t *early_host_SA = nullptr;
    hipStream_t early_stream = nullptr;
    std::vector<hipEvent_t> early_events;
    size_t early_used = 0;
    uint64_t early_bytes = 0;
    void *xf_pin[16][2] = {};
    hipEvent_t xf_done[16][2] = {};
    hipStream_t xf_stream[16] = {};
    int xf_ready = 0;

    uint64_t n = 0, m = 0, m_far = 0;
    uint64_t counts[12] = {0};
    kiss_hip_stats stats{};
    uint64_t profile_mask = 0;
    struct Ev { hipEvent_t a, b; int cls; };
    std::vector<Ev> ev_pool;
    size_t ev_used = 0;
};

void kiss_drain_deferred(kiss_hip_ctx *ctx);
struct KissOwnStreamAtExit {
    kiss_hip_ctx *ctx;
    explicit KissOwnStreamAtExit(kiss_hip_ctx *c) : ctx(c) {}
    ~KissOwnStreamAtExit()
    {
        if (ctx) ctx->stream = ctx->own_stream;
    }
    KissOwnStreamAtExit(const KissOwnStreamAtExit &) = delete;
    KissOwnStreamAtExit &operator=(const KissOwnStreamAtExit &) = delete;
};
struct KissCallStream : KissOwnStreamAtExit {
    KissCallStream(kiss_hip_ctx *c, void *stream) : KissOwnStreamAtExit(c)
    {
        ctx->stream = stream ? (hipStream_t)stream : ctx->own_stream;
        if (!ctx->deferred_free.empty()) kiss_drain_deferred(ctx);
    }
};

struct KTimer {
    kiss_hip_ctx *ctx;
    int idx;
    KTimer(kiss_hip_ctx *c, int cls, uint64_t items);
    ~KTimer();
};
void ktimer_collect(kiss_hip_ctx *ctx);

static inline uint64_t div_up(uint64_t a, uint64_t b) { return (a + b - 1) / b; }

int kiss_lms_reserve(kiss_hip_ctx *ctx, uint64_t m_cap, uint64_t t_cap_wanted = 0, bool defer_frees = false);
int kiss_lms_reserve_deferred(kiss_hip_ctx *ctx, uint64_t m_cap);
int kiss_tied_reserve(kiss_hip_ctx *ctx, uint64_t t_cap);
int kiss_workspace_ready(kiss_hip_ctx *ctx);
int kiss_need_ctx_words(kiss_hip_ctx *ctx);
int kiss_pack_text(kiss_hip_ctx *ctx, const uint8_t *d_S, uint64_t n);
int kiss_classify(kiss_hip_ctx *ctx, uint64_t n, uint64_t depth , uint64_t win_lo, uint64_t win_hi);
int kiss_readback(kiss_hip_ctx *ctx, const void *d_src, uint32_t nwords);
std::mutex &kiss_device_mutex(int device);
int kiss_scan_u32(kiss_hip_ctx *ctx, const uint32_t *in, uint32_t *out, uint64_t count);
int kiss_scan_u64(kiss_hip_ctx *ctx, const uint64_t *in, uint64_t *out, uint64_t count);
int kiss_zero_u32(kiss_hip_ctx *ctx, void *p, uint64_t count_u32);
int kiss_fill_u32(kiss_hip_ctx *ctx, void *p, uint32_t value, uint64_t count_u32);
struct RadixBufs {
    uint64_t *key[2];
    uint32_t *seg[2];
    uint32_t *pos[2];
    const uint32_t *first_pos = nullptr;
};
static inline RadixBufs kiss_ctx_radix_bufs(kiss_hip_ctx *ctx)
{
    RadixBufs b;
    b.key[0] = ctx->keyA;
    b.key[1] = ctx->keyB;
    b.seg[0] = b.seg[1] = nullptr;
    b.pos[0] = ctx->posA;
    b.pos[1] = ctx->posB;
    return b;
}
constexpr int RX_MAX_PASSES = 12;
int kiss_radix_sort(kiss_hip_ctx *ctx, RadixBufs &b, uint64_t count, int key_lo_bit, int seg_bits, int *result_idx);
int kiss_radix_check(kiss_hip_ctx *ctx);
uint64_t kiss_depth_of(uint64_t n, uint32_t k);
int kiss_key_hist(kiss_hip_ctx *ctx, const uint64_t *d_keys, uint64_t count, int bits, uint64_t *d_hist);
int kiss_partition_by_splitters(kiss_hip_ctx *ctx, const uint64_t *d_keys, const uint32_t *d_pos, uint64_t count, int bits,
                                const uint32_t *splitters, int groups, uint64_t *d_keys_out, uint32_t *d_pos_out);
int kiss_lms_sort(kiss_hip_ctx *ctx, uint64_t n, uint32_t k, uint64_t depth);
constexpr uint64_t KISS_EXACT_MSD_MAX_DEPTH = 32768;
constexpr int KISS_INTERNAL_TOO_DEEP = 1000;
constexpr uint32_t KISS_EXACT_H0 = 512;
int kiss_exact_refine(kiss_hip_ctx *ctx, uint64_t n, uint32_t h0, uint32_t *d_SA, uint8_t *heads_in = nullptr);
int kiss_isa_build(kiss_hip_ctx *ctx, const uint32_t *SA, uint64_t total, uint32_t *isa);
int kiss_rank_build_lms(kiss_hip_ctx *ctx, const uint32_t *L, const uint32_t *lms_asc, uint64_t m, uint64_t n,
                        uint32_t *rank, uint64_t *pairs1, uint64_t *pairs2, uint32_t *small, uint64_t small_words);
int kiss_lms_exact_refine(kiss_hip_ctx *ctx, uint64_t n, uint32_t h0, uint32_t *scratch, bool *resolved);
int kiss_merge_lms(kiss_hip_ctx *ctx);
#ifdef KISS_HIP_HOOKS
void kiss_tie_trace_report(kiss_hip_ctx *ctx);
#endif
int kiss_place_lms(kiss_hip_ctx *ctx, uint64_t n, uint32_t k, uint64_t depth);
int kiss_xfer_h2d(kiss_hip_ctx *ctx, void *d_dst, const void *h_src, uint64_t bytes);
int kiss_io_reserve(kiss_hip_ctx *ctx, uint64_t n);
int kiss_cached_ctx_run(int device, uint64_t n, int (*fn)(kiss_hip_ctx *, void *), void *arg);
template <class F>
static inline int kiss_one_shot_cached(int device, uint64_t max_n, const F &f)
{
    return kiss_cached_ctx_run(device, max_n, [](kiss_hip_ctx *ctx, void *p) { return (*static_cast<const F *>(p))(ctx); }, (void *)&f);
}
template <class F>
static inline int kiss_one_shot_own(int device, uint64_t max_n, const F &f)
{
    kiss_hip_ctx *ctx = nullptr;
    int rc = kiss_hip_ctx_create(&ctx, device, max_n);
    if (rc) return rc;
    rc = f(ctx);
    kiss_hip_ctx_destroy(ctx);
    return rc;
}
int kiss_xfer_d2h(kiss_hip_ctx *ctx, void *h_dst, const void *d_src, uint64_t bytes);
void kiss_xfer_free(kiss_hip_ctx *ctx);
int kiss_induce(kiss_hip_ctx *ctx, uint64_t n, uint32_t *d_SA);
int kiss_early_out(kiss_hip_ctx *ctx, const uint32_t *d_SA, uint64_t lo, uint64_t hi);

#ifdef __HIPCC__
__device__ __forceinline__ void kiss_words2(const uint64_t *__restrict__ pk, uint64_t w, uint64_t &a, uint64_t &b)
{
    const uint64_t w0 = w & ~1ull;
    const ulonglong2 ab = *reinterpret_cast<const ulonglong2 *>(__builtin_assume_aligned(pk + w0, 16));
    const uint64_t c = pk[w0 + 2];
    const bool odd = (w & 1ull) != 0;
    a = odd ? ab.y : ab.x;
    b = odd ? c : ab.y;
}
__device__ __forceinline__ void kiss_words5(const uint64_t *__restrict__ pk, uint64_t w, uint64_t x[5])
{
    const uint64_t w0 = w & ~1ull;
    const ulonglong2 p0 = *reinterpret_cast<const ulonglong2 *>(__builtin_assume_aligned(pk + w0, 16));
    const ulonglong2 p1 = *reinterpret_cast<const ulonglong2 *>(__builtin_assume_aligned(pk + w0 + 2, 16));
    const ulonglong2 p2 = *reinterpret_cast<const ulonglong2 *>(__builtin_assume_aligned(pk + w0 + 4, 16));
    const bool odd = (w & 1ull) != 0;
    x[0] = odd ? p0.y : p0.x;
// ... 53 lines not shown
```

kiss_amd/csrc/lms_sort.hip:

```cpp
#include "flag_compact.hpp"
#include <cstdio>
#include <vector>

using namespace kiss_fc;

namespace {

constexpr uint32_t LMS_SMALL_SEG = 24;
constexpr int ROUND0_BASES = 20;

__global__ __launch_bounds__(LS_THREADS) void k_gather_keys(const uint64_t *__restrict__ pk, uint64_t n,
                                                           const uint32_t *__restrict__ pos, uint64_t count,
                                                           uint64_t depth_off, uint64_t mask,
                                                           uint64_t *__restrict__ key, const uint32_t *__restrict__ seg,
                                                           const uint32_t *__restrict__ segstart, uint32_t min_len,
                                                           uint32_t max_len)
{
    uint64_t i = (uint64_t)blockIdx.x * LS_THREADS + threadIdx.x;
    if (i >= count) return;
    if (seg) {
        const uint32_t sg = seg[i];
        const uint32_t len = segstart[sg + 1] - segstart[sg];
        if (len < min_len || len > max_len) return;
    }
// ... 259 lines not shown
    __syncthreads();
    const int nadj = (int)s_nadj;
    for (int e = tid; e < nadj; e += SF_THREADS) {
        const int w = s_adj[e];
        const bool pair = s_b[w] - s_a[w] == 2;
        bool tied = false;
        const bool ok = !deep_less(pk, n, s_pos[w + 1], s_pos[w], pair ? off - 32 : off, depth, false, &tied);
        s_inorder[w] = tied ? 2 : (ok ? 1 : 0);
    }
    __syncthreads();
    for (int w = tid; w < SF_WINDOW; w += SF_THREADS) {
        const int wa = s_a[w], wb = s_b[w];
        bool sorted = true;
        for (int j = wa; j + 1 < wb; j++) sorted = sorted && s_inorder[j] != 0;
        if (sorted) continue;
        s_unsorted[w] = 1;
        const bool own = w >= SF_HALO && w < SF_HALO + SF_THREADS;
        const uint64_t ki = s_key[w];
        uint32_t before = 0, walk = 0;
        for (int j = w + 1; j < wb; j++) {
            const uint64_t kj = s_key[j];
            const uint32_t bit = 1u << (j - w);
            if (kj != ki) before |= ki < kj ? bit : 0u;
            else if (j == w + 1) before |= s_inorder[w] ? bit : 0u;
            else if (own || (j >= SF_HALO && j < SF_HALO + SF_THREADS)) walk |= bit;
        }
        s_before[w] = before;
        if (s_inorder[w] == 2) s_tiedm[w] = 2u;
        if (walk) {
            uint32_t at = atomicAdd(&s_nfar, (uint32_t)__popc(walk));
            while (walk) {
                const int d = __ffs(walk) - 1;
                walk &= walk - 1;
                s_far[at++] = (uint16_t)(w | (d << 9));
            }
        }
    }
    __syncthreads();
    const int nfar = (int)s_nfar;
    for (int e = tid; e < nfar; e += SF_THREADS) {
        const int w = s_far[e] & 511, d = s_far[e] >> 9;
        bool tied = false;
        const bool first = deep_less(pk, n, s_pos[w], s_pos[w + d], off, depth, true, &tied);
        if (first) atomicOr(&s_before[w], 1u << d);
        if (tied) atomicOr(&s_tiedm[w], 1u << d);
    }
    __syncthreads();
    const int w = tid + SF_HALO;
    const uint32_t i = (uint32_t)(g0 + w);
    if (my_len == 0) return;
    if (my_len > LMS_SMALL_SEG) {
        big[i] = i == my_a ? (uint8_t)3 : (uint8_t)1;
        return;
    }
    const int wa = s_a[w], wb = s_b[w];
    uint32_t r;
    bool taint, tied_before;
    if (!s_unsorted[w]) {
        r = (uint32_t)(w - wa);
        tied_before = w > wa && s_inorder[w - 1] == 2;
        taint = tied_before || (w + 1 < wb && s_inorder[w] == 2);
    } else {
        const uint32_t behind = (2u << (wb - 1 - w)) - 2u;
        r = (uint32_t)__popc(~s_before[w] & behind);
        taint = s_tiedm[w] != 0;
        tied_before = false;
        for (int j = wa; j < w; j++) {
            r += (s_before[j] >> (w - j)) & 1u;
            tied_before = tied_before || ((s_tiedm[j] >> (w - j)) & 1u);
        }
        taint = taint || tied_before;
    }
    const uint32_t dst = slot[my_a + r];
    out[dst] = s_pos[w];
    if (hfar && tied_before) hfar[dst] = 0;
    if (tctx) octx[dst] = tctx[i] | (taint ? KISS_CTX_TAINT : 0u);
    else if (taint) octx[dst] = KISS_CTX_TAINT;
    big[i] = 0;
}

__global__ __launch_bounds__(LS_THREADS) void k_pair_finish(const uint64_t *__restrict__ pk, uint64_t n,
                                                           const uint32_t *__restrict__ rpos0,
                                                           const uint32_t *__restrict__ rpos1,
                                                           const uint32_t *__restrict__ rslot, uint64_t npairs,
                                                           uint64_t off, uint64_t depth, uint32_t *__restrict__ out,
                                                           uint32_t *__restrict__ octx, uint8_t *__restrict__ hfar)
{
    const uint64_t i = (uint64_t)blockIdx.x * LS_THREADS + threadIdx.x;
    if (i >= npairs) return;
    const uint32_t p0 = rpos0[i], p1 = rpos1[i], s = rslot[i];
    bool taint = false;
    const bool swap = deep_less(pk, n, p1, p0, off - 32, depth, false, &taint);
    if (!swap && !taint) return;
    const uint32_t c0 = octx[s], c1 = octx[s + 1];
    const uint32_t t = taint ? KISS_CTX_TAINT : 0u;
    if (swap) {
        out[s] = p1;
        out[s + 1] = p0;
    }
    octx[s] = (swap ? c1 : c0) | t;
    octx[s + 1] = (swap ? c0 : c1) | t;
    if (hfar && taint) hfar[s + 1] = 0;
}

__device__ __forceinline__ uint32_t pivot_class(const uint64_t *__restrict__ bkey, uint32_t a, uint32_t b, uint64_t k)
{
    const uint64_t pv = bkey[(a + b) >> 1];
    return k < pv ? 0u : (k == pv ? 1u : 2u);
}

__global__ __launch_bounds__(LS_THREADS) void k_pivot_class(const uint64_t *__restrict__ bkey,
                                                           const uint32_t *__restrict__ bseg,
                                                           const uint32_t *__restrict__ bsegstart, uint64_t nbig,
                                                           uint64_t *__restrict__ cls)
{
    const uint64_t i = (uint64_t)blockIdx.x * LS_THREADS + threadIdx.x;
    if (i >= nbig) return;
    const uint32_t sid = bseg[i];
    const uint32_t c = pivot_class(bkey, bsegstart[sid], bsegstart[sid + 1], bkey[i]);
    cls[i] = c == 0 ? 1ull : (c == 1 ? (1ull << 32) : 0ull);
}

__global__ __launch_bounds__(LS_THREADS) void k_pivot_scatter(const uint64_t *__restrict__ bkey,
                                                             const uint32_t *__restrict__ bpos,
                                                             const uint32_t *__restrict__ bseg,
                                                             const uint32_t *__restrict__ bsegstart, uint64_t nbig,
                                                             const uint64_t *__restrict__ cls,
                                                             const uint64_t *__restrict__ ex,
                                                             const uint64_t *__restrict__ tot,
                                                             uint64_t *__restrict__ okey, uint32_t *__restrict__ opos,
                                                             uint64_t *__restrict__ ne)
{
    const uint64_t i = (uint64_t)blockIdx.x * LS_THREADS + threadIdx.x;
    if (i >= nbig) return;
    const uint32_t sid = bseg[i];
    const uint32_t a = bsegstart[sid], b = bsegstart[sid + 1];
    const uint64_t ea = ex[a], eb = (uint64_t)b < nbig ? ex[b] : tot[0], ei = ex[i], ci = cls[i];
    const uint32_t t0 = (uint32_t)eb - (uint32_t)ea, t1 = (uint32_t)(eb >> 32) - (uint32_t)(ea >> 32);
    const uint32_t lt_before = (uint32_t)ei - (uint32_t)ea, eq_before = (uint32_t)(ei >> 32) - (uint32_t)(ea >> 32);
    const uint32_t c = (uint32_t)ci ? 0u : ((ci >> 32) ? 1u : 2u);
    uint32_t d;
    if (c == 0) d = a + lt_before;
    else if (c == 1) d = a + t0 + eq_before;
    else d = a + t0 + t1 + ((uint32_t)i - a - lt_before - eq_before);
    okey[d] = bkey[i];
    opos[d] = bpos[i];
    uint64_t f = 0;
    if (c == 0) f = (1ull << 32) | (uint64_t)(d == a ? 1u : 0u);
    else if (c == 2) f = (1ull << 32) | (uint64_t)(d == a + t0 + t1 ? 1u : 0u);
    ne[d] = f;
}


__device__ __forceinline__ uint64_t maj3(uint64_t a, uint64_t b, uint64_t c) { return (a & b) | (a & c) | (b & c); }

__global__ __launch_bounds__(LS_THREADS) void k_pivot_lcp(const uint64_t *__restrict__ pk,
                                                         const uint32_t *__restrict__ bpos,
                                                         const uint32_t *__restrict__ bseg,
                                                         const uint32_t *__restrict__ bsegstart, uint64_t nbig,
                                                         uint64_t off, uint64_t depth, int dbits, int slots,
                                                         uint64_t *__restrict__ keyout, int frac_den, int with_ctx)
{
    const uint64_t i = (uint64_t)blockIdx.x * LS_THREADS + threadIdx.x;
    if (i >= nbig) return;
    const uint32_t sid = bseg[i];
    const uint32_t a = bsegstart[sid], b = bsegstart[sid + 1], len = b - a;
    const uint64_t p = (uint64_t)bpos[i] + off;
    const uint64_t f1 = frac_den == 4 ? 1 : (frac_den == 7 ? 2 : 3), f2 = frac_den == 4 ? 2 : (frac_den == 7 ? 4 : 5),
                   f3 = frac_den == 4 ? 3 : (frac_den == 7 ? 5 : 8);
    const uint64_t q1 = (uint64_t)bpos[a + (uint32_t)(((uint64_t)len * f1) / (uint64_t)frac_den)] + off,
                   q2 = (uint64_t)bpos[a + (uint32_t)(((uint64_t)len * f2) / (uint64_t)frac_den)] + off,
                   q3 = (uint64_t)bpos[a + (uint32_t)(((uint64_t)len * f3) / (uint64_t)frac_den)] + off;
// ... 45 lines not shown
        used++;
        complete = true;
    }
    key <<= (uint64_t)slotbits * (uint64_t)(slots - used);
    key = (key << 1) | (complete ? 1ull : 0ull);
    keyout[i] = (key << (64 - (slots * slotbits + 1))) | (with_ctx ? (uint64_t)kiss_load_ctx_n(pk, bpos[i], KISS_KEY_CTX_BASES) : 0ull);
}

__global__ __launch_bounds__(LS_THREADS) void k_pivot_heads(const uint64_t *__restrict__ key,
                                                           const uint32_t *__restrict__ seg, uint64_t nbig,
                                                           int complete_bit, uint8_t *__restrict__ heads,
                                                           uint64_t cmp_mask)
{
    const uint64_t i = (uint64_t)blockIdx.x * LS_THREADS + threadIdx.x;
    if (i >= nbig) return;
    const uint64_t k = key[i] & cmp_mask;
    const bool complete = ((k >> complete_bit) & 1ull) != 0;
    const bool same_prev = i > 0 && seg[i] == seg[i - 1] && (key[i - 1] & cmp_mask) == k;
    uint8_t h = 1;
    if (same_prev && !complete) h = 0;
    if (complete && (same_prev || (i + 1 < nbig && seg[i + 1] == seg[i] && (key[i + 1] & cmp_mask) == k))) h |= 2;
    if (complete && same_prev) h |= 4;
    heads[i] = h;
}

__global__ void k_ctx_lengths_anchor(const uint64_t *pk, uint32_t *out)
{
    out[threadIdx.x] = kiss_load_ctx(pk, out[threadIdx.x + 64]);
}


struct LmsViews {
    uint32_t *rpos0, *rpos1, *rslot;
    uint64_t rcol;
    uint64_t *K1;
    uint64_t *key2;
    uint64_t *F1, *F2;
    uint8_t *pivot_heads;
    uint32_t *seg2, *bss;
    uint32_t *sortpos[2];
    uint32_t *tctx, *bslot;
    uint64_t *d_total, *d_ptot;
    uint32_t *d_nbig;
};

LmsViews views_of(kiss_hip_ctx *ctx)
{
    LmsViews v;
    v.rcol = (ctx->m_far / 2 + 4) & ~3ull;
    v.rpos0 = reinterpret_cast<uint32_t *>(ctx->keyA);
    v.rpos1 = v.rpos0 + v.rcol;
    v.rslot = v.rpos1 + v.rcol;
    v.K1 = ctx->keyA;
    v.key2 = ctx->keyB;
    v.F1 = ctx->flags;
    v.F2 = ctx->flags + ctx->t_cap;
    v.pivot_heads = reinterpret_cast<uint8_t *>(ctx->segB);
    v.seg2 = ctx->segB;
    v.bss = ctx->segstartB;
    v.sortpos[0] = ctx->lmsP;
    v.sortpos[1] = ctx->lmsC;
    v.tctx = v.bslot = ctx->bslot;
    v.d_total = reinterpret_cast<uint64_t *>(ctx->d_small + 2);
    v.d_nbig = ctx->d_small + 8;
    v.d_ptot = reinterpret_cast<uint64_t *>(ctx->d_small + 24);
    return v;
}

struct LmsSort {
    kiss_hip_ctx *ctx;
    uint64_t n, depth;
    bool dbg;
    bool pivot_on;
    bool pivot_r1;
    int pivot_slots;
    bool no_pair_keys;
    uint32_t small_seg;
    bool small_fused;
    LmsViews v;
    uint32_t *Pc, *Sc, *Gc, *SSc;
    uint64_t count, nseg;
    uint64_t off = ROUND0_BASES;
    uint64_t npairs = 0;
    bool have_tctx = false;
    bool first_refine = true;
    unsigned pivot_rounds_done = 0;

    FcOut survivors() const { return FcOut{Pc, Sc, Gc, SSc}; }
    void take_tied_arrays()
    {
        Sc = ctx->slotA;
        Gc = ctx->segA;
        SSc = ctx->segstartA;
        v = views_of(ctx);
    }
    void set_survivors(uint64_t tot)
    {
        count = tot >> 32;
        nseg = tot & 0xFFFFFFFFull;
    }
};

struct Round {
    uint64_t mask;
    int key_lo_bit;
    bool last_round, pivot_ahead;
    unsigned grid;
    uint8_t *inorder, *bigb;
};

Round round_of(const LmsSort &s)
{
    Round r;
    uint64_t rem = s.depth ? s.depth - s.off : 32;
    if (rem > 32) rem = 32;
    r.last_round = s.depth ? (s.off + 32 >= s.depth) : false;
    r.mask = rem >= 32 ? ~0ull : (~0ull << (64 - 2 * rem));
    r.key_lo_bit = (int)(64 - 2 * rem);
    r.grid = (unsigned)div_up(s.count, LS_THREADS);
    r.pivot_ahead = s.depth && (s.off > ROUND0_BASES || s.pivot_r1) && s.pivot_on;
    r.inorder = reinterpret_cast<uint8_t *>(s.v.F2);
    r.bigb = r.inorder + ((s.count + 15) & ~15ull);
    return r;
}

int regrow_tied(LmsSort &s, uint64_t surv)
{
    KTRY(kiss_tied_reserve(s.ctx, surv + surv / 8 + 1024));
    s.take_tied_arrays();
    return KISS_HIP_OK;
}

int round0(LmsSort &s)
{
    kiss_hip_ctx *ctx = s.ctx;
    const uint64_t count = ctx->m_far;
    RadixBufs rb;
    rb.first_pos = ctx->lms_pos;
    rb.key[0] = ctx->keyA;
    rb.key[1] = ctx->keyB;
    rb.pos[0] = ctx->posA;
    static_assert(KISS_R0_PASSES % 2 == 1, "round-0 result must land in buffer 1");
    rb.pos[1] = ctx->lms_sorted_far;
    rb.seg[0] = rb.seg[1] = nullptr;
    const int r0_shift = 64 - 2 * ROUND0_BASES;
    static_assert(64 - 2 * ROUND0_BASES == KISS_R0_SHIFT && (2 * ROUND0_BASES + 7) / 8 == KISS_R0_PASSES, "classify.hip counts these digits");
    int res = 0;
    KTRY(kiss_radix_sort(ctx, rb, count, r0_shift, 0, &res));
    ctx->stats.lms_rounds++;
    ctx->stats.sort_item_rounds += count;
    s.Pc = rb.pos[res ^ 1];
    uint64_t tot;
    const bool onepass = !ctx->opts.no_fc0_onepass && fc0_onepass_fits(ctx, count) && rb.pos[res] == ctx->lms_sorted_far;
    const bool pair_records = onepass && !ctx->opts.no_pair_records && rb.key[res] == ctx->keyB;
    if (onepass) {
        for (int attempt = 0;; attempt++) {
            const Fc0Job job{rb.key[res], rb.pos[res], count, r0_shift, ctx->lms_ctx_far, s.v.tctx,
                             pair_records ? s.v.rpos0 : (uint32_t *)nullptr, (uint32_t)s.v.rcol};
            KTRY(fc0_onepass(ctx, job, s.survivors(), s.v.d_total, &tot, &s.npairs));
            if ((tot >> 32) <= ctx->t_cap) break;
            if (attempt) return KINTERNAL();
            KTRY(regrow_tied(s, tot >> 32));
        }
        s.have_tctx = true;
    } else {
        FcJob job;
        job.key = rb.key[res];
        job.pos = rb.pos[res];
        job.count = count;
        job.cmp_shift = r0_shift;
        job.out = ctx->lms_sorted_far;
        job.octx = ctx->lms_ctx_far;
        KTRY(fc_count(ctx, job, s.v.d_total));
        KTRY(read_u64(ctx, s.v.d_total, &tot));
        if ((tot >> 32) > ctx->t_cap) {
            KTRY(regrow_tied(s, tot >> 32));
            KTRY(fc_count(ctx, job, s.v.d_total));
        }
        job.nctx = s.v.tctx;
        KTRY(fc_compact(ctx, job, s.survivors(), &s.have_tctx));
    }
    s.set_survivors(tot);
    if (s.dbg)
        fprintf(stderr, "[kiss_hip] round 0: items %llu -> survivors %llu in %llu segments\n", (unsigned long long)count,
                (unsigned long long)s.count, (unsigned long long)s.nseg);
    return KISS_HIP_OK;
}

int finish_pair_records(LmsSort &s)
{
    kiss_hip_ctx *ctx = s.ctx;
    if (s.npairs > ctx->m_far / 2) return KINTERNAL();
    {
        KTimer t(ctx, KISS_HIP_K_SEGRANK, 2 * s.npairs);
        hipLaunchKernelGGL(k_pair_finish, dim3((unsigned)div_up(s.npairs, LS_THREADS)), dim3(LS_THREADS), 0, ctx->stream, ctx->pk, s.n,
                           s.v.rpos0, s.v.rpos1, s.v.rslot, s.npairs, (uint64_t)ROUND0_BASES, s.depth, ctx->lms_sorted_far,
                           ctx->lms_ctx_far, ctx->hfar);
        KCHECK(hipGetLastError());
    }
    ctx->stats.pair_records = (uint32_t)s.npairs;
    ctx->stats.sort_item_rounds += 2 * s.npairs;
    if (s.count == 0) ctx->stats.lms_rounds++;
    return KISS_HIP_OK;
}

int gather_keys(LmsSort &s, const Round &r)
{
    kiss_hip_ctx *ctx = s.ctx;
    if (s.small_fused && r.pivot_ahead) return KISS_HIP_OK;
    const uint32_t *seg = s.Gc;
    uint32_t min_len = s.small_seg + 1u, max_len = 0xFFFFFFFFu;
    if (!s.small_fused) {
        seg = s.no_pair_keys ? s.Gc : (const uint32_t *)nullptr;
        min_len = 3u;
        max_len = r.pivot_ahead ? s.small_seg : 0xFFFFFFFFu;
    }
    KTimer t(ctx, KISS_HIP_K_KEYGATHER, s.count);
    set_u32(ctx, s.SSc + s.nseg, (uint32_t)s.count);
    hipLaunchKernelGGL(k_gather_keys, dim3(r.grid), dim3(LS_THREADS), 0, ctx->stream, ctx->pk, s.n, s.Pc, s.count, s.off, r.mask,
                       s.v.K1, seg, s.SSc, min_len, max_len);
    KCHECK(hipGetLastError());
    return KISS_HIP_OK;
}

int finish_small_segments(LmsSort &s, const Round &r)
{
    kiss_hip_ctx *ctx = s.ctx;
    {
        KTimer t(ctx, KISS_HIP_K_SEGRANK, s.count);
        set_u32(ctx, s.SSc + s.nseg, (uint32_t)s.count, s.v.d_nbig);
        const uint32_t *tctx = (s.have_tctx && s.first_refine) ? s.v.tctx : (const uint32_t *)nullptr;
        if (s.small_fused) {
            hipLaunchKernelGGL(k_small_finish, dim3(r.grid), dim3(SF_THREADS), 0, ctx->stream, ctx->pk, s.n, s.Pc, s.Sc, s.Gc, s.SSc,
                               (uint32_t)s.count, s.off, s.depth, r.mask, ctx->lms_sorted_far, r.bigb, tctx, ctx->lms_ctx_far,
                               ctx->hfar);
        } else {
            hipLaunchKernelGGL(k_seg_adjacent, dim3(r.grid), dim3(LS_THREADS), 0, ctx->stream, ctx->pk, s.n, s.v.K1, s.Pc, s.Gc,
                               s.SSc, s.count, s.off, s.depth, s.small_seg, r.inorder);
            hipLaunchKernelGGL(k_seg_finish, dim3(r.grid), dim3(LS_THREADS), 0, ctx->stream, ctx->pk, s.n, s.v.K1, s.Pc, s.Sc, s.Gc,
                               s.SSc, s.count, s.off, s.depth, s.small_seg, r.inorder, ctx->lms_sorted_far, r.bigb, s.v.d_nbig,
                               tctx, ctx->lms_ctx_far, ctx->hfar);
        }
        KCHECK(hipGetLastError());
    }
    ctx->stats.lms_rounds++;
    ctx->stats.sort_item_rounds += s.count;
    return KISS_HIP_OK;
}

int compact_big_segments(LmsSort &s, const Round &r, uint64_t nbig, uint64_t nbigseg)
{
    kiss_hip_ctx *ctx = s.ctx;
    const BigbOut to{ctx->bkeyA, ctx->bposA, ctx->bsegA, s.v.bslot, s.v.bss};
    return bigb_compact(ctx, r.bigb, r.pivot_ahead ? (const uint64_t *)nullptr : s.v.K1, s.Pc, s.Sc, s.count, to, nbig, nbigseg);
}

#ifdef KISS_HIP_HOOKS
int dump_pivot_round(LmsSort &s, const char *dump, uint64_t nbig, uint64_t nbigseg, int dbits, int slots)
{
    kiss_hip_ctx *ctx = s.ctx;
    std::vector<uint32_t> hp(nbig), hs(nbig), hss(nbigseg + 1);
    std::vector<uint64_t> hk(nbig);
    KCHECK(hipStreamSynchronize(ctx->stream));
    KCHECK(hipMemcpy(hp.data(), ctx->bposA, nbig * 4, hipMemcpyDeviceToHost));
    KCHECK(hipMemcpy(hs.data(), ctx->bsegA, nbig * 4, hipMemcpyDeviceToHost));
    KCHECK(hipMemcpy(hss.data(), s.v.bss, (nbigseg + 1) * 4, hipMemcpyDeviceToHost));
    KCHECK(hipMemcpy(hk.data(), ctx->bkeyB, nbig * 8, hipMemcpyDeviceToHost));
    char name[512];
    snprintf(name, sizeof name, "%s.%u", dump, ctx->stats.lms_rounds);
    if (FILE *f = fopen(name, "wb")) {
        const uint64_t hdr[6] = {nbig, nbigseg, s.off, s.depth, (uint64_t)dbits, (uint64_t)slots};
        fwrite(hdr, 8, 6, f);
        fwrite(hp.data(), 4, nbig, f);
        fwrite(hs.data(), 4, nbig, f);
        fwrite(hss.data(), 4, nbigseg + 1, f);
        fwrite(hk.data(), 8, nbig, f);
        fclose(f);
    }
    return KISS_HIP_OK;
}
#endif

int pivot_round(LmsSort &s, uint64_t nbig, uint64_t nbigseg)
{
    kiss_hip_ctx *ctx = s.ctx;
    static const int pivot_den[3] = {4, 7, 11};
    const unsigned bgrid = (unsigned)div_up(nbig, LS_THREADS);
    const int dbits = bits_for(s.depth - s.off);
    int slots = 63 / (dbits + 4);
    if (slots > s.pivot_slots) slots = s.pivot_slots;
    const int kbits = slots * (dbits + 4) + 1;
    const int key_lo = 64 - 8 * ((kbits + 7) / 8);
    const bool with_ctx = key_lo >= 24 && !ctx->opts.no_pivot_ctx;
    {
        KTimer t(ctx, KISS_HIP_K_SEGRANK, nbig);
        hipLaunchKernelGGL(k_pivot_lcp, dim3(bgrid), dim3(LS_THREADS), 0, ctx->stream, ctx->pk, ctx->bposA, ctx->bsegA, s.v.bss, nbig,
                           s.off, s.depth, dbits, slots, ctx->bkeyB, pivot_den[s.pivot_rounds_done % 3], with_ctx ? 1 : 0);
        s.pivot_rounds_done++;
        KCHECK(hipGetLastError());
// ... 84 lines not shown
        b.ex = H2;
        b.nbig = nne;
        b.ngroups = ngroups;
        b.key_lo_bit = r.key_lo_bit;
        b.kbuf[0] = s.v.key2;
        b.kbuf[1] = ctx->bkeyA;
        b.pbuf[0] = s.v.sortpos[0];
        b.pbuf[1] = s.v.sortpos[1];
        b.sbuf[0] = ctx->bsegB;
        b.sbuf[1] = s.v.seg2;
        b.bidx = ctx->bposA;
        b.okey = ctx->bkeyB;
        b.opos = ctx->bposB;
        KTRY(sort_big_members(ctx, b));
    }
    ctx->stats.big_item_rounds += nne;
    *sorted = SortedBig{ctx->bkeyB, ctx->bposB, ctx->bsegA};
    return KISS_HIP_OK;
}

int radix_round(LmsSort &s, const Round &r, uint64_t nbig, uint64_t nbigseg, SortedBig *sorted)
{
    kiss_hip_ctx *ctx = s.ctx;
    RadixBufs bb;
    bb.key[0] = ctx->bkeyA;
    bb.key[1] = ctx->bkeyB;
    bb.pos[0] = ctx->bposA;
    bb.pos[1] = ctx->bposB;
    bb.seg[0] = ctx->bsegA;
    bb.seg[1] = ctx->bsegB;
    int bres = 0;
    KTRY(kiss_radix_sort(ctx, bb, nbig, r.key_lo_bit, bits_for(nbigseg), &bres));
    ctx->stats.big_item_rounds += nbig;
    *sorted = SortedBig{bb.key[bres], bb.pos[bres], bits_for(nbigseg) ? bb.seg[bres] : ctx->bsegA};
    return KISS_HIP_OK;
}

int closing_compaction(LmsSort &s, const Round &r, const SortedBig &sorted, uint64_t nbig)
{
    kiss_hip_ctx *ctx = s.ctx;
    FcJob job;
    job.src = FC_KEY_SEG;
    job.key = sorted.key;
    job.seg = sorted.seg;
    job.pos = sorted.pos;
    job.slot = s.v.bslot;
    job.count = nbig;
    job.last_round = (int)r.last_round;
    job.out = ctx->lms_sorted_far;
    job.tmark = ctx->lms_ctx_far;
    uint64_t tot;
    KTRY(fc_count(ctx, job, s.v.d_total));
    KTRY(fc_compact(ctx, job, s.survivors()));
    KTRY(read_u64(ctx, s.v.d_total, &tot));
    s.set_survivors(tot);
    return KISS_HIP_OK;
}

struct DbgSpan {
    hipStream_t stream;
    hipEvent_t e0 = nullptr, e1 = nullptr;
    DbgSpan(kiss_hip_ctx *ctx, bool on) : stream(ctx->stream)
    {
        if (!on) return;
        (void)hipEventCreate(&e0);
        (void)hipEventCreate(&e1);
        (void)hipEventRecord(e0, stream);
    }
    float ms()
    {
        float v = 0;
        (void)hipEventRecord(e1, stream);
        (void)hipEventSynchronize(e1);
        (void)hipEventElapsedTime(&v, e0, e1);
        return v;
    }
    ~DbgSpan()
    {
        if (e0) (void)hipEventDestroy(e0);
        if (e1) (void)hipEventDestroy(e1);
    }
};

}

int kiss_lms_sort(kiss_hip_ctx *ctx, uint64_t n, uint32_t k, uint64_t depth)
{
    (void)k;
    const uint64_t m_far = ctx->m_far;
    ctx->stats.lms_rounds = 0;
    ctx->stats.sort_item_rounds = 0;
    ctx->stats.pair_records = 0;
    if (m_far == 0) return KISS_HIP_OK;
    if (m_far == 1) {
        KCHECK(hipMemcpyAsync(ctx->lms_sorted_far, ctx->lms_pos, sizeof(uint32_t), hipMemcpyDeviceToDevice,
                              ctx->stream));
        KTRY(kiss_zero_u32(ctx, ctx->lms_ctx_far, 1));
        return KISS_HIP_OK;
    }
    LmsSort s;
    s.ctx = ctx;
    s.n = n;
    s.depth = depth;
    s.dbg = ctx->opts.debug;
    s.pivot_on = !ctx->opts.no_pivot_rounds;
    s.pivot_r1 = !ctx->opts.pivot_from_round2;
    s.pivot_slots = ctx->opts.pivot_slots >= 1 && ctx->opts.pivot_slots <= 8 ? ctx->opts.pivot_slots : 3;
    s.no_pair_keys = !ctx->opts.pair_keys;
    s.small_seg = ctx->opts.small_seg >= 2 && ctx->opts.small_seg <= 4096 ? ctx->opts.small_seg : LMS_SMALL_SEG;
    s.small_fused = !ctx->opts.no_small_fused && s.small_seg == LMS_SMALL_SEG;
    s.take_tied_arrays();

    KTRY(round0(s));
    if (s.npairs) KTRY(finish_pair_records(s));

    for (;; s.first_refine = false) {
        if (s.count == 0) break;
        if (depth && s.off >= depth) return KINTERNAL();
        const Round r = round_of(s);
        KTRY(gather_keys(s, r));
        uint64_t bt;
        {
            DbgSpan span(ctx, s.dbg);
            KTRY(finish_small_segments(s, r));
            KTRY(bigb_count(ctx, r.bigb, s.count, s.v.d_total, &bt));
            if (s.dbg) fprintf(stderr, "[kiss_hip]   seg_finish + flag scan %.3f ms\n", span.ms());
        }
        const uint64_t nbig = bt >> 32, nbigseg = bt & 0xFFFFFFFFull;
        if (s.dbg)
            fprintf(stderr, "[kiss_hip] round off=%llu: items %llu in %llu segments, big-segment items %llu\n",
                    (unsigned long long)s.off, (unsigned long long)s.count, (unsigned long long)s.nseg, (unsigned long long)nbig);
        if (nbig == 0) break;
        KTRY(compact_big_segments(s, r, nbig, nbigseg));
        if (r.pivot_ahead) {
            KTRY(pivot_round(s, nbig, nbigseg));
            continue;
        }
        SortedBig sorted;
        if (uint64_t *NE = class_split_flags(s, nbig)) KTRY(class_split_round(s, r, NE, nbig, nbigseg, &sorted));
        else KTRY(radix_round(s, r, nbig, nbigseg, &sorted));
        KTRY(closing_compaction(s, r, sorted, nbig));
        s.off += 32;
        if (!depth && s.off > n + 64 && s.count > 0) return KINTERNAL();
        if (!depth && s.off >= KISS_EXACT_MSD_MAX_DEPTH && s.count > 0) return KISS_INTERNAL_TOO_DEEP;
    }
    return KISS_HIP_OK;
}
```

kiss_amd/sorter.py:

```python
import ctypes

import numpy as np

from . import _lib

K_UNBOUNDED = 0xFFFFFFFF


_CTX_LIB = {}


def _check(status, where, ctx=None):
    if status != _lib.KISS_HIP_OK:
        detail = ""
        if ctx is not None:
            msg = ctypes.c_char_p()
            lib = _CTX_LIB.get(getattr(ctx, "value", ctx)) or _lib.load()
            code = lib.kiss_hip_last_hip_error(ctx, ctypes.byref(msg))
            if code:
                detail = "hip error %d: %s" % (code, (msg.value or b"").decode())
        raise _lib.KissHipError(status, where, detail)


class Context:

    def __init__(self, max_n, device=0, profiling=False, lms_capacity=0, hooks=None):
        self._lib = _lib.load(hooks)
        self._ctx = ctypes.c_void_p()
        _check(self._lib.kiss_hip_ctx_create_sized(ctypes.byref(self._ctx), int(device), int(max_n), int(lms_capacity)),
               "kiss_hip_ctx_create_sized")
        _CTX_LIB[self._ctx.value] = self._lib
        self._owned = True
        self.max_n = int(max_n)
        self.device = int(device)
        if profiling:
            self.set_profiling(True)

    @classmethod
    def _borrowed(cls, handle, max_n, device):
        self = cls.__new__(cls)
        self._lib = _lib.load()
        self._ctx = ctypes.c_void_p(handle)
        self._owned = False
        self.max_n, self.device = int(max_n), int(device)
        return self

    def close(self):
        if self._ctx and self._owned:
            _CTX_LIB.pop(self._ctx.value, None)
            self._lib.kiss_hip_ctx_destroy(self._ctx)
        self._ctx = ctypes.c_void_p()

    def release_io_buffers(self):
        _check(self._lib.kiss_hip_ctx_release_io_buffers(self._ctx), "kiss_hip_ctx_release_io_buffers", self._ctx)

    def __enter__(self):
        return self

    def __exit__(self, *a):
        self.close()

    def __del__(self):
        try:
            self.close()
        except Exception:
            pass

    def load_text_file(self, path):
        d_S = ctypes.c_void_p()
        n = ctypes.c_uint64()
        _check(self._lib.kiss_hip_ctx_load_text_file(self._ctx, str(path).encode(), ctypes.byref(d_S), ctypes.byref(n)),
               "kiss_hip_ctx_load_text_file", self._ctx)
        return d_S.value, n.value

    def free_dev(self, ptr):
        if ptr:
            _check(self._lib.kiss_hip_free_dev(ctypes.c_void_p(ptr)), "kiss_hip_free_dev")

    def read_sequence(self, path):
        ptr, n = self.load_text_file(path)
        try:
            out = np.empty(n, dtype=np.uint8)
            if n:
                _check(self._lib.kiss_hip_copy_to_host(out.ctypes.data, ctypes.c_void_p(ptr), n), "kiss_hip_copy_to_host")
        finally:
            self.free_dev(ptr)
        return out

    def set_profiling(self, on, classes=None):
        if on and classes is not None:
            mask = 0
            for c in classes:
                mask |= 1 << _lib.KERNEL_CLASSES.index(c)
            _check(self._lib.kiss_hip_ctx_set_profiling_mask(self._ctx, mask), "kiss_hip_ctx_set_profiling_mask")
        else:
            _check(self._lib.kiss_hip_ctx_set_profiling(self._ctx, 1 if on else 0), "kiss_hip_ctx_set_profiling")

    def workspace_bytes(self):
        v = ctypes.c_uint64()
        _check(self._lib.kiss_hip_ctx_workspace_bytes(self._ctx, ctypes.byref(v)), "kiss_hip_ctx_workspace_bytes")
        return v.value

    def stats(self):
        st = _lib.Stats()
        _check(self._lib.kiss_hip_get_stats(self._ctx, ctypes.byref(st)), "kiss_hip_get_stats")
        return st.as_dict()

    def suffix_sort(self, S, k=256, algo=_lib.ALGO_PARALLEL_SORTING):
        S = np.ascontiguousarray(S, dtype=np.uint8)
        n = S.size
        SA = np.empty(n + 1, dtype=np.uint32)
        _check(self._lib.kiss_hip_ctx_suffix_sort_dna_u32(self._ctx, S.ctypes.data, n, int(k) & 0xFFFFFFFF, int(algo),
                                                          SA.ctypes.data), "kiss_hip_ctx_suffix_sort_dna_u32", self._ctx)
        return SA

    def suffix_sort_host(self, S, SA, k=256, algo=_lib.ALGO_PARALLEL_SORTING):
        assert S.dtype == np.uint8 and SA.dtype == np.uint32 and SA.size == S.size + 1
        assert S.flags["C_CONTIGUOUS"] and SA.flags["C_CONTIGUOUS"]
        _check(self._lib.kiss_hip_ctx_suffix_sort_dna_u32(self._ctx, S.ctypes.data, S.size, int(k) & 0xFFFFFFFF, int(algo),
                                                          SA.ctypes.data), "kiss_hip_ctx_suffix_sort_dna_u32", self._ctx)
        return SA

    def suffix_sort_dev(self, d_S_ptr, n, d_SA_ptr, k=256, algo=_lib.ALGO_PARALLEL_SORTING, stream=None):
        _check(self._lib.kiss_hip_ctx_suffix_sort_dna_u32_dev(self._ctx, ctypes.c_void_p(d_S_ptr), int(n),
                                                              int(k) & 0xFFFFFFFF, int(algo), ctypes.c_void_p(d_SA_ptr),
                                                              ctypes.c_void_p(stream or 0)),
               "kiss_hip_ctx_suffix_sort_dna_u32_dev", self._ctx)

    def verify_sa_dev(self, d_S_ptr, n, d_SA_ptr, k=256, stream=None):
        rep = _lib.VerifyReport()
        _check(self._lib.kiss_hip_ctx_verify_sa_dev(self._ctx, ctypes.c_void_p(d_S_ptr), int(n), int(k) & 0xFFFFFFFF,
                                                    ctypes.c_void_p(d_SA_ptr), ctypes.byref(rep),
                                                    ctypes.c_void_p(stream or 0)), "kiss_hip_ctx_verify_sa_dev", self._ctx)
        return rep.as_dict()

    def lcp_dev(self, d_S_ptr, n, d_SA_ptr, d_LCP_ptr, alphabet="dna", stream=None):
        fn = {"dna": "kiss_hip_ctx_lcp_dna_u32_dev", "bytes": "kiss_hip_ctx_lcp_u8_dev"}[alphabet]
        rep = _lib.LcpReport()
        _check(getattr(self._lib, fn)(self._ctx, ctypes.c_void_p(d_S_ptr), int(n), ctypes.c_void_p(d_SA_ptr),
                                      ctypes.c_void_p(d_LCP_ptr), ctypes.byref(rep), ctypes.c_void_p(stream or 0)),
               fn, self._ctx)
        return rep.as_dict()

    def stage_outputs(self):
        st = self.stats()
        m = st["m"]
        asc = np.empty(m, dtype=np.uint32)
        srt = np.empty(m, dtype=np.uint32)
        counts = np.zeros(12, dtype=np.uint64)
        _check(self._lib.kiss_hip_ctx_get_stage_outputs(self._ctx, asc.ctypes.data, srt.ctypes.data,
                                                        counts.ctypes.data), "kiss_hip_ctx_get_stage_outputs", self._ctx)
        return asc, srt, counts


class MultiContext:

    def __init__(self, devices, max_n):
        self._lib = _lib.load()
        self._mc = ctypes.c_void_p()
        self.devices = [int(d) for d in devices]
        arr = (ctypes.c_int * len(self.devices))(*self.devices)
        _check(self._lib.kiss_hip_multi_create(ctypes.byref(self._mc), arr, len(self.devices), int(max_n)),
               "kiss_hip_multi_create")
        self.max_n = int(max_n)

    def close(self):
        if self._mc:
            self._lib.kiss_hip_multi_destroy(self._mc)
            self._mc = ctypes.c_void_p()

    def __enter__(self):
        return self

    def __exit__(self, *a):
        self.close()

    def __del__(self):
        try:
            self.close()
        except Exception:
            pass

    def rank_context(self, rank=0):
        h = self._lib.kiss_hip_multi_ctx(self._mc, int(rank))
        if not h:
            raise IndexError("no such share")
        return Context._borrowed(h, self.max_n, self.devices[rank])

    def suffix_sort(self, S, k=256, algo=_lib.ALGO_PARALLEL_SORTING):
# ... 92 lines not shown
```

Before: 48.25 billion bases/s.

## Fill host readback spin-waits with deferred chunked pair-finish and induce-count kernels

Adds a fill queue of deferred, chunkable GPU work. One chunk is launched each time the host publishes a readback and spins waiting for it, so the GPU stays busy during those synchronous waits. Pair-record finishing in the LMS sort and the induce count passes (LMS and L-part, computed ahead into a new ind_pre buffer) are moved into this queue and flushed before their results are needed. This adds a second counts buffer and lambda and queue bookkeeping. It also risks ordering bugs, and the early-issued count kernels could compete with critical-path work.

```diff
diff --git a/include/kiss_hip.h b/include/kiss_hip.h
--- a/include/kiss_hip.h
+++ b/include/kiss_hip.h
@@ -181,6 +181,7 @@
                                   int key_lo_bit, int seg_bits, unsigned flags);
 int kiss_hip_debug_scan_u32(kiss_hip_ctx *ctx, uint32_t *data, uint64_t count);
 int kiss_hip_debug_fail_alloc_over(kiss_hip_ctx *ctx, uint64_t bytes);
+int kiss_hip_debug_fill_stats(const kiss_hip_ctx *ctx, uint64_t *out8);
 int kiss_hip_debug_splitters(const uint64_t *hist, uint64_t bins, int groups, uint32_t *splitters_out,
                              uint64_t *group_counts_out);
 
diff --git a/kiss_amd/_lib.py b/kiss_amd/_lib.py
--- a/kiss_amd/_lib.py
+++ b/kiss_amd/_lib.py
@@ -371,6 +371,9 @@
     lib.kiss_hip_stage_reserve.argtypes = [vp, ctypes.c_uint64]
     lib.kiss_hip_debug_fail_alloc_over.argtypes = [vp, ctypes.c_uint64]
     lib.kiss_hip_debug_fail_alloc_over.restype = ctypes.c_int
+    if hasattr(lib, "kiss_hip_debug_fill_stats"):
+        lib.kiss_hip_debug_fill_stats.argtypes = [vp, ctypes.POINTER(ctypes.c_uint64 * 8)]
+        lib.kiss_hip_debug_fill_stats.restype = ctypes.c_int
     lib.kiss_hip_debug_splitters.argtypes = [vp, ctypes.c_uint64, ctypes.c_int, vp, vp]
     lib.kiss_hip_debug_splitters.restype = ctypes.c_int
     lib.kiss_hip_ctx_destroy.argtypes = [vp]
@@ -589,6 +592,7 @@
     "kiss_hip_fmi_chain_dev", "kiss_hip_fmi_chain_host", "kiss_hip_fmi_align_dev", "kiss_hip_fmi_align_host",
     "kiss_hip_fmi_select_dev", "kiss_hip_fmi_select_host", "kiss_hip_fmi_pair_dev", "kiss_hip_fmi_pair_host",
     "kiss_hip_fmi_rescue_dev", "kiss_hip_fmi_rescue_host", "kiss_hip_fmi_aln_merge_dev", "kiss_hip_fmi_aln_merge_host",
+    "kiss_hip_debug_fill_stats",
 ]
 
 READS_EXPORTED_SYMBOLS = [
diff --git a/kiss_amd/csrc/api.hip b/kiss_amd/csrc/api.hip
--- a/kiss_amd/csrc/api.hip
+++ b/kiss_amd/csrc/api.hip
@@ -89,6 +89,9 @@
     o.isa_direct_max = env_u64("KISS_HIP_ISA_DIRECT_MAX", 0);
     o.lx_sync_points = (unsigned)env_u64("KISS_HIP_LX_SYNC_POINTS", 0);
     o.tie_trace = (unsigned)env_u64("KISS_HIP_TIE_TRACE", 0);
+    o.no_fill = (uint32_t)env_u64("KISS_HIP_NO_FILL", 0);
+    o.fill_chunk = env_u64("KISS_HIP_FILL_CHUNK", 0);
+    o.fill_scale = (uint32_t)env_u64("KISS_HIP_FILL_SCALE", 0);
     o.poison = (uint32_t)env_u64("KISS_HIP_POISON", 0);
     if (const char *e = getenv("KISS_HIP_DUMP_PIVOT")) snprintf(o.dump_pivot, sizeof o.dump_pivot, "%s", e);
     ctx->opts = o;
@@ -144,6 +147,7 @@
     const uint32_t seq = ++ctx->pub_seq ? ctx->pub_seq : ++ctx->pub_seq;
     hipLaunchKernelGGL(k_publish, dim3(1), dim3(64), 0, ctx->stream, (const uint32_t *)d_src, nwords, ctx->d_pub, seq);
     KCHECK(hipGetLastError());
+    if (!ctx->fill.empty()) KTRY(ctx->fill.issue_chunk());
     volatile uint32_t *flag = ctx->h_pub + 16;
     const auto t0 = std::chrono::steady_clock::now();
     for (uint64_t spins = 0;; spins++) {
@@ -164,6 +168,41 @@
     return KISS_HIP_OK;
 }
 
+bool kiss_fill_on(const kiss_hip_ctx *ctx, int kind)
+{
+    return !(ctx->opts.no_fill & (1u | (2u << kind))) && !ctx->opts.sync_readback && ctx->h_pub && ctx->d_pub;
+}
+
+int kiss_fill_add(kiss_hip_ctx *ctx, int kind, uint64_t units, uint64_t chunk, uint32_t due,
+                  std::function<int(uint64_t, uint64_t)> launch,
+                  uint64_t *id)
+{
+    if (ctx->opts.fill_scale) chunk = chunk * ctx->opts.fill_scale / 100;
+    if (ctx->opts.fill_chunk) chunk = ctx->opts.fill_chunk;
+    *id = ctx->fill.add(kind, units, chunk, due, std::move(launch));
+    if (!kiss_fill_on(ctx, kind)) return ctx->fill.flush(*id);
+    return KISS_HIP_OK;
+}
+
+int kiss_fill_flush(kiss_hip_ctx *ctx, uint64_t id) { return ctx->fill.flush(id); }
+
+KissFillScope::KissFillScope(kiss_hip_ctx *c) : ctx(c) { ctx->fill.clear(); }
+KissFillScope::~KissFillScope() { ctx->fill.clear(); }
+int KissFillScope::finish() { return ctx->fill.flush_all(); }
+
+int kiss_hip_debug_fill_stats(const kiss_hip_ctx *ctx, uint64_t *out8)
+{
+    if (!ctx || !out8) return KISS_HIP_E_INVALID;
+    const KissFillStats &f = ctx->fill.stats;
+    for (int k = 0; k < KISS_FILL_KINDS; k++) {
+        out8[4 * k + 0] = f.units[k];
+        out8[4 * k + 1] = f.chunks[k];
+        out8[4 * k + 2] = f.issued[k];
+        out8[4 * k + 3] = f.flushed[k];
+    }
+    return KISS_HIP_OK;
+}
+
 bool kiss_host_is_pinned(const void *p);
 void *kiss_prefault_start(kiss_hip_ctx *ctx, void *p, uint64_t bytes);
 void kiss_prefault_join(void *handle);
@@ -241,7 +280,7 @@
 {
     kiss_drain_deferred(ctx);
     free_lms_side(ctx);
-    void *ptrs[] = {ctx->pk, ctx->tile_gp, ctx->tile_cnt, ctx->cl_part, ctx->d_counts, ctx->CTX, ctx->CLS, ctx->ind_counts, ctx->ind_desc,
+    void *ptrs[] = {ctx->pk, ctx->tile_gp, ctx->tile_cnt, ctx->cl_part, ctx->d_counts, ctx->CTX, ctx->CLS, ctx->ind_counts, ctx->ind_pre, ctx->ind_desc,
                     ctx->d_small, ctx->near_idx, ctx->near_fin, ctx->near_pos, ctx->near_tmp, ctx->near_tmp2, ctx->pairs1, ctx->pairs2, ctx->rx_ctl, ctx->refine_heads, ctx->ga_codes};
     for (void *p : ptrs)
         if (p) (void)hipFree(p);
@@ -670,6 +709,8 @@
         ALLOC(cl_part, (ctx->n_tiles_cap < 8192 ? ctx->n_tiles_cap : 8192) * (uint64_t)(KISS_R0_PASSES * 256));
         ALLOC(d_counts, 16);
         ALLOC(ind_counts, ctx->ind_tiles_cap);
+        ctx->ind_pre_cap = 4 * (3 * ((max_n + 1) / 4096 + 1) + 8) + 32;
+        ALLOC(ind_pre, ctx->ind_pre_cap);
         ctx->ind_desc_stride = (max_n + 1) / 1024 + 2;
         ALLOC(ind_desc, 4 * ctx->ind_desc_stride);
         if (hipMemset(ctx->ind_desc, 0, 4 * ctx->ind_desc_stride * sizeof(uint64_t)) != hipSuccess) {
diff --git a/kiss_amd/csrc/fill_queue.hpp b/kiss_amd/csrc/fill_queue.hpp
--- /dev/null
+++ b/kiss_amd/csrc/fill_queue.hpp
@@ -0,0 +1,90 @@
+#pragma once
+#include <cstdint>
+#include <deque>
+#include <functional>
+
+enum { KISS_FILL_PAIRS = 0, KISS_FILL_COUNTS = 1, KISS_FILL_KINDS = 2 };
+
+struct KissFillJob {
+    uint64_t id = 0;
+    int kind = 0;
+    uint64_t next = 0, end = 0;
+    uint64_t chunk = 1;
+    uint32_t due = 0;
+    std::function<int(uint64_t, uint64_t)> launch;
+};
+
+struct KissFillStats {
+    uint64_t units[KISS_FILL_KINDS];
+    uint64_t chunks[KISS_FILL_KINDS];
+    uint64_t issued[KISS_FILL_KINDS];
+    uint64_t flushed[KISS_FILL_KINDS];
+};
+
+struct KissFillQueue {
+    std::deque<KissFillJob> jobs;
+    uint64_t last_id = 0;
+    KissFillStats stats{};
+
+    bool empty() const { return jobs.empty(); }
+    void clear() { jobs.clear(); }
+    void reset_stats(int kind)
+    {
+        stats.units[kind] = stats.chunks[kind] = stats.issued[kind] = stats.flushed[kind] = 0;
+    }
+    uint64_t add(int kind, uint64_t units, uint64_t chunk, uint32_t due, std::function<int(uint64_t, uint64_t)> launch)
+    {
+        const uint64_t id = ++last_id;
+        stats.units[kind] += units;
+        if (units == 0) return id;
+        KissFillJob j;
+        j.id = id;
+        j.kind = kind;
+        j.end = units;
+        j.chunk = chunk ? chunk : 1;
+        j.due = due;
+        j.launch = std::move(launch);
+        auto it = jobs.begin();
+        while (it != jobs.end() && it->due <= due) ++it;
+        jobs.insert(it, std::move(j));
+        return id;
+    }
+    int issue_chunk()
+    {
+        if (jobs.empty()) return 0;
+        KissFillJob &j = jobs.front();
+        const uint64_t a = j.next, left = j.end - j.next;
+        const uint64_t b = a + (j.chunk < left ? j.chunk : left);
+        j.next = b;
+        stats.chunks[j.kind]++;
+        stats.issued[j.kind] += b - a;
+        const int rc = j.launch(a, b);
+        if (rc != 0) {
+            clear();
+            return rc;
+        }
+        if (jobs.front().next == jobs.front().end) jobs.pop_front();
+        return 0;
+    }
+    int flush(uint64_t id)
+    {
+        for (auto it = jobs.begin(); it != jobs.end(); ++it) {
+            if (it->id != id) continue;
+            KissFillJob j = std::move(*it);
+            jobs.erase(it);
+            stats.flushed[j.kind] += j.end - j.next;
+            const int rc = j.launch(j.next, j.end);
+            if (rc != 0) clear();
+            return rc;
+        }
+        return 0;
+    }
+    int flush_all()
+    {
+        while (!jobs.empty()) {
+            const int rc = flush(jobs.front().id);
+            if (rc != 0) return rc;
+        }
+        return 0;
+    }
+};
diff --git a/kiss_amd/csrc/induce.hip b/kiss_amd/csrc/induce.hip
--- a/kiss_amd/csrc/induce.hip
+++ b/kiss_amd/csrc/induce.hip
@@ -266,12 +266,13 @@
 __global__ __launch_bounds__(IN_THREADS) void k_induce_count(const uint64_t *__restrict__ pk, const uint32_t *srcP,
                                                             uint32_t *srcC, int64_t beg, uint64_t N, int dir,
                                                             uint32_t emitmask, uint32_t *__restrict__ counts,
-                                                            uint64_t tiles, LmsRemap rm, uint8_t *srcK)
-{
-    if (blockIdx.x == 0 && threadIdx.x == 4) counts[4 * tiles] = 0;
+                                                            uint64_t tiles, LmsRemap rm, uint8_t *srcK,
+                                                            uint64_t tile0, uint64_t tile1)
+{
+    if (tile0 == 0 && blockIdx.x == 0 && threadIdx.x == 4) counts[4 * tiles] = 0;
     const uint32_t wave = (uint32_t)__builtin_amdgcn_readfirstlane((int)(threadIdx.x >> 6));
-    const uint64_t tile = (uint64_t)blockIdx.x * IN_WAVES + wave;
-    if (tile >= tiles) return;
+    const uint64_t tile = tile0 + (uint64_t)blockIdx.x * IN_WAVES + wave;
+    if (tile >= tile1) return;
     const uint64_t t0 = tile * IN_TILE;
     int64_t shift = 0;
     bool block = t0 + IN_TILE <= N;
@@ -758,8 +759,75 @@
     int64_t pos[4];
 };
 
+struct CountSrc {
+    const uint32_t *srcP;
+    uint32_t *srcC;
+    int64_t beg;
+    uint64_t N;
+    int dir;
+    uint32_t emitmask;
+    bool remap;
+    LmsRemap rm;
+    uint8_t *srcK;
+};
+
+uint8_t *class_bytes_of(kiss_hip_ctx *ctx, const uint32_t *srcC)
+{
+    return (srcC == ctx->CTX && ctx->CLS && !ctx->opts.no_class_bytes && !ctx->opts.induce_one_pass) ? ctx->CLS : nullptr;
+}
+
+uint64_t small_max_of(const kiss_hip_ctx *ctx)
+{
+    return ctx->opts.induce_small_max >= 64 && ctx->opts.induce_small_max <= (1u << 20) ? ctx->opts.induce_small_max : (uint64_t)SMALL_MAX;
+}
+
+int launch_count(kiss_hip_ctx *ctx, const CountSrc &cs, uint32_t *counts, uint64_t tiles, uint64_t a, uint64_t b)
+{
+    if (a >= b || b > tiles) return KINTERNAL();
+    const uint64_t i0 = a * IN_TILE, i1 = b * IN_TILE < cs.N ? b * IN_TILE : cs.N;
+    KTimer t(ctx, KISS_HIP_K_INDUCE_COUNT, i1 - i0);
+    const dim3 grid((unsigned)div_up(b - a, IN_WAVES));
+    if (cs.remap)
+        hipLaunchKernelGGL(k_induce_count<true>, grid, dim3(IN_THREADS), 0, ctx->stream, ctx->pk, cs.srcP, cs.srcC, cs.beg, cs.N,
+                           cs.dir, cs.emitmask, counts, tiles, cs.rm, cs.srcK, a, b);
+    else
+        hipLaunchKernelGGL(k_induce_count<false>, grid, dim3(IN_THREADS), 0, ctx->stream, ctx->pk, cs.srcP, cs.srcC, cs.beg, cs.N,
+                           cs.dir, cs.emitmask, counts, tiles, cs.rm, cs.srcK, a, b);
+    KCHECK(hipGetLastError());
+    return KISS_HIP_OK;
+}
+
+struct PreCount {
+    uint64_t job = 0;
+    uint32_t *counts = nullptr;
+    uint64_t tiles = 0;
+};
+
+constexpr uint64_t PRE_CHUNK_LMS = 4096, PRE_CHUNK_LPART = 16384;
+
+struct PreCounts {
+    kiss_hip_ctx *ctx;
+    uint64_t used = 0;
+    int add(const CountSrc &cs, uint64_t chunk, uint32_t due, PreCount *pc)
+    {
+        *pc = PreCount{};
+        if (!kiss_fill_on(ctx, KISS_FILL_COUNTS) || ctx->opts.induce_one_pass || !ctx->ind_pre) return KISS_HIP_OK;
+        if (cs.N <= small_max_of(ctx) || cs.emitmask == 0) return KISS_HIP_OK;
+        const uint64_t tiles = div_up(cs.N, IN_TILE), words = (4 * tiles + 1 + 3) & ~3ull;
+        if (used + words > ctx->ind_pre_cap) return KISS_HIP_OK;
+        uint32_t *counts = ctx->ind_pre + used;
+        used += words;
+        kiss_hip_ctx *c = ctx;
+        pc->counts = counts;
+        pc->tiles = tiles;
+        return kiss_fill_add(ctx, KISS_FILL_COUNTS, tiles, chunk, due, [c, cs, counts, tiles](uint64_t a, uint64_t b) -> int {
+            return launch_count(c, cs, counts, tiles, a, b);
+        }, &pc->job);
+    }
+};
+
 int run_pass(Sweep &sw, const uint32_t *srcP, uint32_t *srcC, int64_t beg, uint64_t N, uint32_t emitmask,
-             int selfclass, uint64_t tot[4], bool *chain_done, const LmsRemap *remap = nullptr)
+             int selfclass, uint64_t tot[4], bool *chain_done, const LmsRemap *remap = nullptr, const PreCount *pre = nullptr)
 {
     kiss_hip_ctx *ctx = sw.ctx;
     const LmsRemap rm = remap ? *remap : LmsRemap{nullptr, nullptr, 0u};
@@ -773,10 +841,10 @@
     DstPos dp;
     for (int c = 0; c < 4; c++) dp.p[c] = sw.pos[c];
     ctx->stats.induce_passes++;
-    uint8_t *const srcK = (srcC == ctx->CTX && ctx->CLS && !ctx->opts.no_class_bytes && !ctx->opts.induce_one_pass) ? ctx->CLS : nullptr;
-    const uint64_t small_max = ctx->opts.induce_small_max >= 64 && ctx->opts.induce_small_max <= (1u << 20) ? ctx->opts.induce_small_max
-                                                                                                           : (uint64_t)SMALL_MAX;
+    uint8_t *const srcK = class_bytes_of(ctx, srcC);
+    const uint64_t small_max = small_max_of(ctx);
     if (N <= small_max) {
+        if (pre && pre->counts) return KINTERNAL();
         {
             KTimer t(ctx, KISS_HIP_K_INDUCE_SMALL, N);
             if (remap)
@@ -810,28 +878,27 @@
         } else
 #endif
         {
-        {
-            KTimer t(ctx, KISS_HIP_K_INDUCE_COUNT, N);
-            if (remap)
-                hipLaunchKernelGGL(k_induce_count<true>, dim3((unsigned)div_up(tiles, IN_WAVES)), dim3(IN_THREADS), 0, ctx->stream,
-                                   ctx->pk, srcP, srcC, beg, N, sw.dir, emitmask, ctx->ind_counts, tiles, rm, srcK);
-            else
-                hipLaunchKernelGGL(k_induce_count<false>, dim3((unsigned)div_up(tiles, IN_WAVES)), dim3(IN_THREADS), 0, ctx->stream,
-                                   ctx->pk, srcP, srcC, beg, N, sw.dir, emitmask, ctx->ind_counts, tiles, rm, srcK);
-            KCHECK(hipGetLastError());
-        }
-        KTRY(kiss_scan_u32(ctx, ctx->ind_counts, ctx->ind_counts, 4 * tiles + 1));
+        uint32_t *counts = ctx->ind_counts;
+        if (pre && pre->counts) {
+            if (pre->tiles != tiles) return KINTERNAL();
+            KTRY(kiss_fill_flush(ctx, pre->job));
+            counts = pre->counts;
+        } else {
+            const CountSrc cs{srcP, srcC, beg, N, sw.dir, emitmask, remap != nullptr, rm, srcK};
+            KTRY(launch_count(ctx, cs, counts, tiles, 0, tiles));
+        }
+        KTRY(kiss_scan_u32(ctx, counts, counts, 4 * tiles + 1));
         {
             KTimer t(ctx, KISS_HIP_K_INDUCE_SCATTER, N);
             if (remap)
                 hipLaunchKernelGGL((k_induce_scatter<true, 1>), dim3((unsigned)tiles), dim3(IN_THREADS), 0, ctx->stream, ctx->pk, srcP,
-                                   srcC, beg, N, emitmask, ctx->ind_counts, tiles, dp, sw.SA, ctx->CTX, ctx->d_small, rm, ctx->CLS, srcK);
+                                   srcC, beg, N, emitmask, counts, tiles, dp, sw.SA, ctx->CTX, ctx->d_small, rm, ctx->CLS, srcK);
             else if (sw.dir > 0)
                 hipLaunchKernelGGL((k_induce_scatter<false, 1>), dim3((unsigned)tiles), dim3(IN_THREADS), 0, ctx->stream, ctx->pk, srcP,
-                                   srcC, beg, N, emitmask, ctx->ind_counts, tiles, dp, sw.SA, ctx->CTX, ctx->d_small, rm, ctx->CLS, srcK);
+                                   srcC, beg, N, emitmask, counts, tiles, dp, sw.SA, ctx->CTX, ctx->d_small, rm, ctx->CLS, srcK);
             else
                 hipLaunchKernelGGL((k_induce_scatter<false, -1>), dim3((unsigned)tiles), dim3(IN_THREADS), 0, ctx->stream, ctx->pk, srcP,
-                                   srcC, beg, N, emitmask, ctx->ind_counts, tiles, dp, sw.SA, ctx->CTX, ctx->d_small, rm, ctx->CLS, srcK);
+                                   srcC, beg, N, emitmask, counts, tiles, dp, sw.SA, ctx->CTX, ctx->d_small, rm, ctx->CLS, srcK);
             KCHECK(hipGetLastError());
         }
         }
@@ -1154,6 +1221,8 @@
 int kiss_induce(kiss_hip_ctx *ctx, uint64_t n, uint32_t *d_SA)
 {
     ctx->stats.induce_passes = 0;
+    KissFillScope fill(ctx);
+    ctx->fill.reset_stats(KISS_FILL_COUNTS);
     KTRY(kiss_need_ctx_words(ctx));
     ctx->ctx_words_valid = false;
     uint64_t cnt[4], cntS[4], cntL[4], cntLMS[4], start[5], lms_start[5];
@@ -1184,6 +1253,15 @@
     if (collapse_max > ctx->t_cap) collapse_max = ctx->t_cap;
 
     const LmsRemap lms_rm{ctx->rm_fin, ctx->rm_pos, ctx->rm_E};
+    PreCounts pre{ctx};
+    PreCount pre_lms[4], pre_lpart[4];
+    for (int c = 0; c < 4; c++) {
+        const uint32_t mask_gt = (0xFu << (c + 1)) & 0xFu;
+        const CountSrc cs = ctx->lms_merged
+            ? CountSrc{ctx->lmsP, ctx->lmsC, (int64_t)lms_start[c], cntLMS[c], +1, mask_gt, false, LmsRemap{nullptr, nullptr, 0u}, nullptr}
+            : CountSrc{ctx->lms_sorted_far, ctx->lms_ctx_far, (int64_t)lms_start[c], cntLMS[c], +1, mask_gt, true, lms_rm, nullptr};
+        KTRY(pre.add(cs, PRE_CHUNK_LMS, (uint32_t)c, &pre_lms[c]));
+    }
     Sweep L{ctx, d_SA, +1, {(int64_t)start[0], (int64_t)start[1], (int64_t)start[2], (int64_t)start[3]}};
     KTRY(run_pass(L, seed, seed + 1, 0, 1, 0xFu, -1, tot, &done));
     for (int c = 0; c < 4; c++) {
@@ -1203,8 +1281,13 @@
         KTRY(kiss_early_out(ctx, d_SA, c == 0 ? 0 : start[c], start[c] + cntL[c]));
         if (cntLMS[c]) {
             const uint32_t mask_gt = (0xFu << (c + 1)) & 0xFu;
-            if (ctx->lms_merged) KTRY(run_pass(L, ctx->lmsP, ctx->lmsC, (int64_t)lms_start[c], cntLMS[c], mask_gt, -1, tot, &done));
-            else KTRY(run_pass(L, ctx->lms_sorted_far, ctx->lms_ctx_far, (int64_t)lms_start[c], cntLMS[c], mask_gt, -1, tot, &done, &lms_rm));
+            if (ctx->lms_merged) KTRY(run_pass(L, ctx->lmsP, ctx->lmsC, (int64_t)lms_start[c], cntLMS[c], mask_gt, -1, tot, &done, nullptr, &pre_lms[c]));
+            else KTRY(run_pass(L, ctx->lms_sorted_far, ctx->lms_ctx_far, (int64_t)lms_start[c], cntLMS[c], mask_gt, -1, tot, &done, &lms_rm, &pre_lms[c]));
+        }
+        if (cntL[c] && c > 0) {
+            const CountSrc cs{d_SA, ctx->CTX, (int64_t)(start[c] + cntL[c]) - 1, cntL[c], -1, (1u << c) - 1u, false,
+                              LmsRemap{nullptr, nullptr, 0u}, class_bytes_of(ctx, ctx->CTX)};
+            KTRY(pre.add(cs, PRE_CHUNK_LPART, 8u - (uint32_t)c, &pre_lpart[c]));
         }
     }
 
@@ -1233,9 +1316,10 @@
         KTRY(kiss_early_out(ctx, d_SA, start[c] + cntL[c], start[c + 1]));
         if (cntL[c] && c > 0) {
             const uint32_t mask_lt = (1u << c) - 1u;
-            KTRY(run_pass(S, d_SA, ctx->CTX, (int64_t)(start[c] + cntL[c]) - 1, cntL[c], mask_lt, -1, tot, &done));
-        }
-    }
+            KTRY(run_pass(S, d_SA, ctx->CTX, (int64_t)(start[c] + cntL[c]) - 1, cntL[c], mask_lt, -1, tot, &done, nullptr, &pre_lpart[c]));
+        }
+    }
+    KTRY(fill.finish());
     ctx->ctx_words_valid = true;
     return KISS_HIP_OK;
 }
diff --git a/kiss_amd/csrc/kiss_internal.hpp b/kiss_amd/csrc/kiss_internal.hpp
--- a/kiss_amd/csrc/kiss_internal.hpp
+++ b/kiss_amd/csrc/kiss_internal.hpp
@@ -49,9 +49,13 @@
     uint64_t isa_direct_max = 0;
     unsigned lx_sync_points = 0;
     unsigned tie_trace = 0;
+    uint32_t no_fill = 0;
+    uint64_t fill_chunk = 0;
+    uint32_t fill_scale = 0;
     uint32_t poison = 0;
     char dump_pivot[256] = {0};
 };
+#include "fill_queue.hpp"
 struct kiss_hip_ctx;
 #ifdef KISS_HIP_HOOKS
 void kiss_opts_refresh(kiss_hip_ctx *ctx);
@@ -223,6 +227,8 @@
     bool ctx_words_valid = false;
     uint32_t *ind_counts = nullptr;
     uint64_t ind_tiles_cap = 0;
+    uint32_t *ind_pre = nullptr;
+    uint64_t ind_pre_cap = 0;
     uint64_t *ind_desc = nullptr;
     uint64_t ind_desc_stride = 0, ind_epoch = 0;
     uint32_t ind_ticket_base = 0;
@@ -231,6 +237,7 @@
     uint32_t *h_pub = nullptr;
     uint32_t *d_pub = nullptr;
     uint32_t pub_seq = 0;
+    KissFillQueue fill;
     int pub_mode = -1;
     uint64_t *pairs1 = nullptr, *pairs2 = nullptr;
     uint64_t pairs_cap = 0;
@@ -310,6 +317,17 @@
 int kiss_pack_text(kiss_hip_ctx *ctx, const uint8_t *d_S, uint64_t n);
 int kiss_classify(kiss_hip_ctx *ctx, uint64_t n, uint64_t depth , uint64_t win_lo, uint64_t win_hi);
 int kiss_readback(kiss_hip_ctx *ctx, const void *d_src, uint32_t nwords);
+bool kiss_fill_on(const kiss_hip_ctx *ctx, int kind);
+int kiss_fill_add(kiss_hip_ctx *ctx, int kind, uint64_t units, uint64_t chunk, uint32_t due,
+                  std::function<int(uint64_t, uint64_t)> launch,
+                  uint64_t *id);
+int kiss_fill_flush(kiss_hip_ctx *ctx, uint64_t id);
+struct KissFillScope {
+    kiss_hip_ctx *ctx;
+    explicit KissFillScope(kiss_hip_ctx *c);
+    ~KissFillScope();
+    int finish();
+};
 std::mutex &kiss_device_mutex(int device);
 int kiss_scan_u32(kiss_hip_ctx *ctx, const uint32_t *in, uint32_t *out, uint64_t count);
 int kiss_scan_u64(kiss_hip_ctx *ctx, const uint64_t *in, uint64_t *out, uint64_t count);
diff --git a/kiss_amd/csrc/lms_sort.hip b/kiss_amd/csrc/lms_sort.hip
--- a/kiss_amd/csrc/lms_sort.hip
+++ b/kiss_amd/csrc/lms_sort.hip
@@ -365,12 +365,13 @@
 __global__ __launch_bounds__(LS_THREADS) void k_pair_finish(const uint64_t *__restrict__ pk, uint64_t n,
                                                            const uint32_t *__restrict__ rpos0,
                                                            const uint32_t *__restrict__ rpos1,
-                                                           const uint32_t *__restrict__ rslot, uint64_t npairs,
+                                                           const uint32_t *__restrict__ rslot, uint64_t first,
+                                                           uint64_t end,
                                                            uint64_t off, uint64_t depth, uint32_t *__restrict__ out,
                                                            uint32_t *__restrict__ octx, uint8_t *__restrict__ hfar)
 {
-    const uint64_t i = (uint64_t)blockIdx.x * LS_THREADS + threadIdx.x;
-    if (i >= npairs) return;
+    const uint64_t i = first + (uint64_t)blockIdx.x * LS_THREADS + threadIdx.x;
+    if (i >= end) return;
     const uint32_t p0 = rpos0[i], p1 = rpos1[i], s = rslot[i];
     bool taint = false;
     const bool swap = deep_less(pk, n, p1, p0, off - 32, depth, false, &taint);
@@ -582,6 +583,7 @@
     uint64_t count, nseg;
     uint64_t off = ROUND0_BASES;
     uint64_t npairs = 0;
+    uint64_t pair_job = 0;
     bool have_tctx = false;
     bool first_refine = true;
     unsigned pivot_rounds_done = 0;
@@ -687,17 +689,22 @@
     return KISS_HIP_OK;
 }
 
+constexpr uint64_t PAIR_FILL_CHUNK = 192 * 1024;
+
 int finish_pair_records(LmsSort &s)
 {
     kiss_hip_ctx *ctx = s.ctx;
     if (s.npairs > ctx->m_far / 2) return KINTERNAL();
-    {
-        KTimer t(ctx, KISS_HIP_K_SEGRANK, 2 * s.npairs);
-        hipLaunchKernelGGL(k_pair_finish, dim3((unsigned)div_up(s.npairs, LS_THREADS)), dim3(LS_THREADS), 0, ctx->stream, ctx->pk, s.n,
-                           s.v.rpos0, s.v.rpos1, s.v.rslot, s.npairs, (uint64_t)ROUND0_BASES, s.depth, ctx->lms_sorted_far,
+    const LmsViews v = s.v;
+    const uint64_t n = s.n, depth = s.depth;
+    KTRY(kiss_fill_add(ctx, KISS_FILL_PAIRS, s.npairs, PAIR_FILL_CHUNK, 0, [ctx, v, n, depth](uint64_t a, uint64_t b) -> int {
+        KTimer t(ctx, KISS_HIP_K_SEGRANK, 2 * (b - a));
+        hipLaunchKernelGGL(k_pair_finish, dim3((unsigned)div_up(b - a, LS_THREADS)), dim3(LS_THREADS), 0, ctx->stream, ctx->pk, n,
+                           v.rpos0, v.rpos1, v.rslot, a, b, (uint64_t)ROUND0_BASES, depth, ctx->lms_sorted_far,
                            ctx->lms_ctx_far, ctx->hfar);
         KCHECK(hipGetLastError());
-    }
+        return KISS_HIP_OK;
+    }, &s.pair_job));
     ctx->stats.pair_records = (uint32_t)s.npairs;
     ctx->stats.sort_item_rounds += 2 * s.npairs;
     if (s.count == 0) ctx->stats.lms_rounds++;
@@ -715,6 +722,7 @@
         min_len = 3u;
         max_len = r.pivot_ahead ? s.small_seg : 0xFFFFFFFFu;
     }
+    KTRY(kiss_fill_flush(ctx, s.pair_job));
     KTimer t(ctx, KISS_HIP_K_KEYGATHER, s.count);
     set_u32(ctx, s.SSc + s.nseg, (uint32_t)s.count);
     hipLaunchKernelGGL(k_gather_keys, dim3(r.grid), dim3(LS_THREADS), 0, ctx->stream, ctx->pk, s.n, s.Pc, s.count, s.off, r.mask,
@@ -965,6 +973,8 @@
     }
 };
 
+int lms_rounds(LmsSort &s);
+
 }
 
 int kiss_lms_sort(kiss_hip_ctx *ctx, uint64_t n, uint32_t k, uint64_t depth)
@@ -994,6 +1004,20 @@
     s.small_fused = !ctx->opts.no_small_fused && s.small_seg == LMS_SMALL_SEG;
     s.take_tied_arrays();
 
+    KissFillScope fill(ctx);
+    ctx->fill.reset_stats(KISS_FILL_PAIRS);
+    const int rc = lms_rounds(s);
+    if (rc != KISS_HIP_OK && rc != KISS_INTERNAL_TOO_DEEP) return rc;
+    KTRY(fill.finish());
+    return rc;
+}
+
+namespace {
+
+int lms_rounds(LmsSort &s)
+{
+    kiss_hip_ctx *ctx = s.ctx;
+    const uint64_t n = s.n, depth = s.depth;
     KTRY(round0(s));
     if (s.npairs) KTRY(finish_pair_records(s));
 
@@ -1029,3 +1053,5 @@
     }
     return KISS_HIP_OK;
 }
+
+}
diff --git a/kiss_amd/sorter.py b/kiss_amd/sorter.py
--- a/kiss_amd/sorter.py
+++ b/kiss_amd/sorter.py
@@ -105,6 +105,12 @@
         st = _lib.Stats()
         _check(self._lib.kiss_hip_get_stats(self._ctx, ctypes.byref(st)), "kiss_hip_get_stats")
         return st.as_dict()
+
+    def fill_stats(self):
+        v = (ctypes.c_uint64 * 8)()
+        _check(self._lib.kiss_hip_debug_fill_stats(self._ctx, ctypes.byref(v)), "kiss_hip_debug_fill_stats")
+        names = ("units", "chunks", "issued", "flushed")
+        return {kind: {nm: int(v[4 * i + j]) for j, nm in enumerate(names)} for i, kind in enumerate(("pairs", "counts"))}
 
     def suffix_sort(self, S, k=256, algo=_lib.ALGO_PARALLEL_SORTING):
         S = np.ascontiguousarray(S, dtype=np.uint8)
```

Result: no change. 47.82 billion bases/s (-0.9%).
